# cai4cai/torchsparsegradutils

Hardware: AMD Instinct MI355X
Metric: CSR SpMM+SDDMM achieved HBM GB/s (algorithmic bytes), N=1e6 nnz/row=27 RHS=32, fwd+bwd (higher is better)
Workload: dtype f32

## Files before the change

### include/tsgu_hip.h

```cpp
#ifndef TSGU_HIP_H
#define TSGU_HIP_H

#include <stdint.h>

#ifdef __cplusplus
extern "C" {
#endif

#define TSGU_ABI_VERSION 7

typedef enum {
    TSGU_OK = 0,
    TSGU_ERR_BAD_DTYPE = -1,
    TSGU_ERR_BAD_ARG = -2,
    TSGU_ERR_TOO_LARGE = -3,
    TSGU_ERR_LAUNCH = -4,
    TSGU_ERR_RUNTIME = -5,
    TSGU_ERR_RESERVED_6 = -6,
    TSGU_ERR_TIMEOUT = -7
} tsgu_status;

typedef enum { TSGU_F32 = 0, TSGU_F64 = 1, TSGU_BF16 = 2 } tsgu_vtype;
typedef enum { TSGU_I32 = 0, TSGU_I64 = 1 } tsgu_itype;

int tsgu_abi_version(void);
const char* tsgu_status_string(int status);
int tsgu_device_info(int device, char* name, int cap, int* n_cu, int* wave_size);
int tsgu_device_cu_count(int device, int* n_cu);
int tsgu_device_copy(const void* src, void* dst, int64_t bytes, int device, void* stream);

int tsgu_index_fingerprint(int itype, int64_t n, const void* x, void* out2, int accumulate, int device, void* stream);
int tsgu_index_fingerprint_match(int itype, int64_t n, const void* x, const void* ref, void* copy, void* out3, int accumulate,
                                 int device, void* stream);

int tsgu_csr_spmm(int vtype, int itype,
                  int64_t n_rows, int64_t n_cols, int64_t nnz_per_item,
                  const void* crow, const void* col, const void* val, const void* perm,
                  const void* B, int64_t ldb, int64_t b_col_stride, int64_t b_batch_stride,
                  void* C, int64_t ldc, int64_t c_col_stride, int64_t c_batch_stride,
                  int64_t p, int64_t batch, int64_t max_row_nnz,
                  const void* dot_w, int64_t ldw, void* dot_partial,
                  int device, void* stream);

int64_t tsgu_spmm_num_blocks(int vtype, int64_t n_rows, int64_t nnz_per_item, int64_t p, int64_t max_row_nnz);

int tsgu_csr_geometry(int kernel, int vtype, int64_t n_rows, int64_t nnz_per_item, int64_t p, int64_t max_row_nnz,
                      int wide_ok, int col_strided,
                      int* vec, int* column_lanes, int* entry_lanes, int64_t* column_tiles, int* row_runs, int* stage_entries);

int tsgu_csr_sddmm(int vtype, int itype,
                   int64_t n_rows, int64_t n_cols, int64_t nnz_per_item,
                   const void* crow, const void* col,
                   const void* G, int64_t ldg, int64_t g_batch_stride,
                   const void* B, int64_t ldb, int64_t b_batch_stride,
                   void* out, double alpha, int swap_roles,
                   int64_t p, int64_t batch,
                   int device, void* stream);

int tsgu_coo_sddmm(int vtype, int itype, int64_t nnz,
                   const void* row, const void* col,
                   const void* G, int64_t ldg, const void* B, int64_t ldb,
                   void* out, double alpha, int64_t p,
                   int device, void* stream);

int tsgu_csr_mm_backward(int vtype, int itype, int64_t n_rows, int64_t n_cols, int64_t nnz_per_item,
                         const void* t_ptr, const void* t_idx, const void* t_perm, const void* val,
                         const void* G, int64_t ldg, int64_t g_batch_stride,
                         const void* B, int64_t ldb, int64_t b_batch_stride,
                         void* gradA_vals, void* gradB, int64_t ldgb, int64_t gb_batch_stride,
                         int64_t p, int64_t batch, int device, void* stream);

typedef struct tsgu_rowpack_plan {
    int64_t nblocks;
    int32_t ecap, ucap;
    int32_t nclasses;
    int32_t rows_per_group;
    const void* uptr;
    const void* ucol;
    const void* upos;
    const void* sperm;
    const void* order;
    const void* vpair;
    const void* eptr;
    const void* wcls;
    const void* wbase;
    const void* cne;
    const void* srcstart;
} tsgu_rowpack_plan;

int tsgu_rowpack_geometry(int vtype, int64_t p, int* rows_per_block, int* entry_lanes, int* max_entries, int* max_union,
                          int* lds_budget_bytes);
int tsgu_csr_spmm_rowpack(int vtype, int itype, int64_t n_rows, int64_t n_cols, int64_t nnz, const void* ptr,
                          const tsgu_rowpack_plan* plan, const void* val, const void* B, int64_t ldb, void* C, int64_t ldc,
                          int64_t p, int device, void* stream);
int tsgu_csr_mm_backward_rowpack(int vtype, int itype, int64_t n_rows_t, int64_t n_cols_t, int64_t nnz, const void* t_ptr,
                                 const tsgu_rowpack_plan* plan, const void* val, const void* G, int64_t ldg, const void* B,
                                 int64_t ldb, void* gradA_vals, void* gradB, int64_t ldgb, int64_t p, int device, void* stream);
int tsgu_csr_sddmm_rowpack(int vtype, int itype, int64_t n_rows, int64_t n_cols, int64_t nnz, const void* ptr,
                           const tsgu_rowpack_plan* plan, const void* R, int64_t ldr, const void* Cm, int64_t ldc,
                           void* out_vals, double alpha, int64_t p, int device, void* stream);

typedef struct tsgu_tile_plan {
    int64_t n_rows, n_cols, nnz;
    int64_t n_blocks;
    int32_t rows_per_block, max_union, max_entries, reserved;
    const void* desc;
    const void* ucol;
    const void* lidx;
    const void* rptr;
    const void* cpos;
    const void* cslot;
    const void* ent;
    const void* xrow;
} tsgu_tile_plan;

int tsgu_tile_geometry(int vtype, int64_t p, int* rows_per_block, int* max_union, int* max_entries);
int tsgu_csr_spmm_tile(int vtype, const tsgu_tile_plan* plan, const void* val, const void* B, int64_t ldb, void* C, int64_t ldc,
                       int64_t p, int device, void* stream);
int tsgu_csr_sddmm_tile(int vtype, const tsgu_tile_plan* plan, const void* R, int64_t ldr, const void* Cm, int64_t ldc, void* out_vals,
                        double alpha, int64_t p, int device, void* stream);

typedef struct tsgu_lattice_plan {
    int32_t kind;
    int32_t nb, nx, ny, nz;
    int32_t ry, rz;
    int32_t ncls, recw;
    int32_t nloc;
    int32_t uniform_len;
    int32_t ty, tz;
    int32_t nseg;
    int32_t threads;
    int32_t ring;
    int32_t chunks_per_lane;
    const void* rec;
    const void* lens;
    const void* rcls;
    const void* rstart;
    const void* wlist;
} tsgu_lattice_plan;

int tsgu_lattice_lds_bytes(int mode, int vtype, int64_t p, int ty, int tz, int ry, int rz, int nloc, int recw, int threads, int ring,
                           int chunks_per_lane);
int tsgu_csr_spmm_lattice(int vtype, const tsgu_lattice_plan* plan, int64_t n_rows, int64_t nnz, const void* val,
                          const void* B, int64_t ldb, void* C, int64_t ldc, int64_t p, int device, void* stream);
int tsgu_csr_spmm_lattice_dot(int vtype, const tsgu_lattice_plan* plan, int64_t n_rows, int64_t nnz, const void* val,
                              const void* B, int64_t ldb, void* C, int64_t ldc, int64_t p, void* dot_partial, int64_t dot_rows,
                              const int* skip, const void* dot_w, int device, void* stream);
int tsgu_csr_sddmm_lattice(int vtype, const tsgu_lattice_plan* plan, int64_t n_rows, int64_t nnz, const void* R, int64_t ldr,
                           const void* Cm, int64_t ldc, void* out_vals, double alpha, int64_t p, int device, void* stream);

typedef struct tsgu_march_plan {
    int32_t nb, nx, ny, nz;
    int32_t ry, rz;
    int32_t ntap;
    int32_t tap_dy[9], tap_dz[9];
    int32_t ncls, ident;
    int32_t ty, tz;
    int32_t nseg;
    int32_t threads;
    uint32_t mask;
    int32_t periodic;
    int32_t uniform_len;
    const void* kidx;
    const void* rcls;
    const void* rstart;
} tsgu_march_plan;

int tsgu_march_supported(int mode, int mask, int uniform_len, int threads);
int tsgu_march_lds_bytes(int mode, int vtype, int64_t p, int ty, int tz, int ry, int rz, int ncls, int threads);
int tsgu_csr_spmm_march(int vtype, const tsgu_march_plan* plan, int transposed, int64_t n_rows, int64_t nnz, const void* val,
                        const void* B, int64_t ldb, void* C, int64_t ldc, int64_t p, int device, void* stream);
int tsgu_csr_sddmm_march(int vtype, const tsgu_march_plan* plan, int64_t n_rows, int64_t nnz, const void* R, int64_t ldr,
                         const void* Cm, int64_t ldc, void* out_vals, double alpha, int accumulate, int64_t p, int device,
                         void* stream);

int tsgu_lattice_slots(void);
int tsgu_lattice_rows(int itype, int64_t n_rows, const void* crow, const void* col, int nb, int nx, int ny, int nz, const void* disp, int nd,
                      void* slot, void* thash, void* trep, const void* remap, const void* ctable, const void* lens, void* rcls, void* status,
                      int box_mask, int periodic, int device, void* stream);
int tsgu_lattice_row_codes(int itype, int64_t n_rows, const void* crow, const void* col, int nb, int nx, int ny, int nz, const void* disp,
                           int nd, const void* rows, int nrows, void* out, int device, void* stream);
int tsgu_lattice_block_classes(int64_t n_rows, const void* rcls, int nb, int nx, int ny, int nz, int ty, int tz, int nseg, void* mask,
                               int device, void* stream);

int tsgu_csr_sptrsm(int vtype, int itype,
                    int64_t n, int64_t nnz,
                    const void* ptr, const void* idx, const void* perm, const void* val,
                    int lower, int unit,
                    const void* B, int64_t ldb, int64_t b_col_stride, void* X, int64_t ldx, int64_t p,
                    void* work, int workgroups_per_cu, int device, void* stream);
int64_t tsgu_sptrsm_work_bytes(int64_t n, int64_t p);

typedef struct {
    int32_t kind, nlines, nz, ncls, width, uniform_len, front_lines, reserved;
    const void* tab;
    const void* lens;
    const void* rcls;
    const void* rstart;
} tsgu_trsm_lattice_plan;
int tsgu_csr_sptrsm_lattice(int vtype, const tsgu_trsm_lattice_plan* plan, int64_t nnz, const void* val,
                            int lower, int unit,
                            const void* B, int64_t ldb, int64_t b_col_stride, void* X, int64_t ldx, int64_t p,
                            void* work, int workgroups, int device, void* stream);

int64_t tsgu_cg_fold_rows(void);
int tsgu_cg_alpha(int vtype, const void* pap_partial, int64_t n_partial, void* fold, void* scal, int* flags,
                  double eps, int64_t p, int device, void* stream);
int tsgu_cg_update1(int vtype, int64_t n, int64_t p,
                    void* r, const void* Ap, void* x, const void* pvec,
                    const void* scal, const int* flags, void* rr_partial,
                    int device, void* stream);
int tsgu_cg_update1_alpha(int vtype, int64_t n, int64_t p, void* r, const void* Ap, void* x, const void* pvec, const void* pap_partial,
                          int64_t n_partial, void* scal, const int* flags, double eps, void* rr_partial, int device, void* stream);
int64_t tsgu_cg2_num_blocks(int vtype, int64_t n, int64_t p);
int tsgu_cg2_residual(int vtype, int64_t n, int64_t p, void* r, const void* Ap, const void* pap_partial, int64_t n_partial, void* scal2,
                      const int* flags2, int parity, double eps, void* rr_partial, int device, void* stream);
int tsgu_cg2_direction(int vtype, int64_t n, int64_t p, const void* r, void* pvec, void* x, const void* rr_partial, int64_t n_partial,
                       void* scal2, int* flags2, int parity, double eps, double stop_updating_after, double tolerance,
                       int min_iter_index, void* hist, int n_hist, int device, void* stream);
int64_t tsgu_cg_num_blocks(int vtype, int64_t n, int64_t p);
int tsgu_cg_beta(int vtype, const void* rr_partial, int64_t n_partial, void* scal, int* flags,
                 double eps, double stop_updating_after, double tolerance, int iter_index,
                 int min_iter_index, int64_t p, int device, void* stream);
int tsgu_cg_beta_precond(int vtype, const void* rr_partial, int64_t n_partial, const void* rz_partial, int64_t n_rz, void* scal,
                         int* flags, double eps, double stop_updating_after, double tolerance, int iter_index,
                         int min_iter_index, int64_t p, int device, void* stream);
int tsgu_cg_update2(int vtype, int64_t n, int64_t p, const void* r, void* pvec,
                    const void* scal, const int* flags, int device, void* stream);

int tsgu_bicg_scalar(int vtype, int phase, const void* partial, int64_t n_partial, int64_t set_stride, void* fold,
                     void* scal, int* flags, double abstol, double reltol, int matvec_max, int nmv0, int64_t p,
                     int device, void* stream);
int tsgu_bicg_vector(int vtype, int which, int64_t n, int64_t p, void* a0, void* a1, const void* a2, const void* a3,
                     const void* a4, const void* scal, const int* flags, void* partial, int64_t set_stride,
                     int device, void* stream);
int tsgu_bicg_update_x_precond(int vtype, int64_t n, int64_t p, void* x, void* r, const void* s, const void* t,
                               const void* q, const void* z, const void* scal, const int* flags, void* partial,
                               int device, void* stream);

int tsgu_minres_scalar(int vtype, int phase, const void* partial, int64_t n_partial, int64_t set_stride, void* fold,
                       void* scal, int* flags, double eps, double tol, double shift, int64_t p, int device, void* stream);
int tsgu_minres_vector(int vtype, int which, int64_t n, int64_t p, void* a0, const void* a1, void* a2, const void* a3,
                       void* a4, const void* scal, const int* flags, void* partial, int64_t set_stride, int with_norms,
                       int device, void* stream);
int tsgu_minres_scalar_ms(int vtype, int phase, const void* partial, int64_t n_partial, int64_t set_stride, void* fold,
                          void* scal, int* flags, double eps, double tol, const void* shifts, int n_shift, double value,
                          int64_t p, int device, void* stream);
int tsgu_minres_vector_ms(int vtype, int which, int64_t n, int64_t p, void* a0, const void* a1, void* a2, const void* a3,
                          void* a4, void* qc, const void* scal, const int* flags, void* partial, int64_t set_stride,
                          int with_norms, int n_shift, int64_t shift_stride, double value, int device, void* stream);

int64_t tsgu_coldot_max_blocks(int64_t n, int64_t p);
int tsgu_coldot(int vtype, int64_t n, int64_t p, const void* X, int64_t ldx,
                const void* Y, int64_t ldy, void* partial, void* out,
                int device, void* stream);

int tsgu_segment_logsumexp_workspace(int vtype, int64_t nnz, int64_t* bytes_host);
int tsgu_segment_logsumexp(int vtype, int itype, int64_t n_groups, int64_t nnz, const void* ptr, const void* perm,
                           const void* val, int include_zeros, int64_t axis_len, void* out, int64_t groups_per_item,
                           int64_t item_stride, void* workspace, int64_t workspace_bytes, int device, void* stream);
int tsgu_segment_logsumexp_backward(int vtype, int itype, int64_t nnz, const void* val, const void* ptr, int64_t n_groups,
                                    const void* g_grp, const void* lse_grp, const void* idx, const void* g_idx,
                                    const void* lse_idx, void* grad, int device, void* stream);

int tsgu_segment_mm_tile_rows(void);
int tsgu_segment_mm(int vtype, int itype, int64_t n, int64_t d1, int64_t d2, int64_t n_seg, const void* offsets,
                    const void* tile_ptr, int64_t max_tiles, const void* perm, const void* a, int64_t lda, const void* b,
                    int64_t b_stride0, int64_t b_stride1, int64_t b_stride2, void* out, int64_t ldo, int device, void* stream);
int tsgu_segment_mm_grad_b_workspace(int vtype, int64_t n, int64_t n_seg, int64_t d1, int64_t d2, int64_t* chunk_rows,
                                     int64_t* max_chunks, int64_t* bytes);
int tsgu_segment_mm_grad_b(int vtype, int itype, int64_t n, int64_t d1, int64_t d2, int64_t n_seg, const void* offsets,
                           const void* chunk_ptr, const void* part_ptr, int64_t chunk_rows, int64_t max_chunks, const void* perm,
                           const void* a, int64_t lda, const void* g, int64_t ldg, void* grad_b, void* workspace,
                           int64_t workspace_bytes, int device, void* stream);

int64_t tsgu_mvn_reduce_blocks(int64_t rows_per_item);
int tsgu_csr_diag_positions(int itype, int64_t n_rows, int64_t nnz, const void* crow, const void* col, const void* perm,
                            void* pos, int device, void* stream);
int tsgu_diag_logsum(int vtype, int itype, int64_t n_rows, int64_t rows_per_item, int64_t n_val, const void* pos,
                     const void* val, void* out, void* partial, int64_t partial_elems, int device, void* stream);
int tsgu_diag_logsum_backward(int vtype, int itype, int64_t n_rows, int64_t rows_per_item, int64_t nnz, const void* crow,
                              const void* perm, const void* pos, const void* val, const void* g, void* grad, int fill,
                              int device, void* stream);
int tsgu_quadform(int vtype, int64_t n, int64_t k, const void* Y, int64_t ldy, int64_t y_col_stride, const void* E,
                  int64_t lde, int64_t e_col_stride, const void* w, int w_mode, int64_t rows_per_item, void* out,
                  void* partial, int64_t partial_elems, int device, void* stream);
int tsgu_quadform_backward(int vtype, int64_t n, int64_t k, const void* Y, int64_t ldy, int64_t y_col_stride, const void* E,
                           int64_t lde, int64_t e_col_stride, const void* w, int w_mode, int64_t rows_per_item, const void* g,
                           void* grad_Y, int64_t ldg, int64_t g_col_stride, void* grad_w, int device, void* stream);
int tsgu_csr_row_sumsq(int vtype, int itype, int64_t n_rows, int64_t nnz, int64_t n_w, const void* crow, const void* col,
                       const void* perm, const void* val, const void* w, const void* add, void* out, int device,
                       void* stream);
int tsgu_csr_row_sumsq_backward(int vtype, int itype, int64_t n_rows, int64_t nnz, int64_t n_w, const void* crow,
                                const void* col, const void* perm, const void* val, const void* w, const void* g, void* grad_val,
                                int device, void* stream);

#ifdef __cplusplus
}
#endif
#endif
```

### torchsparsegradutils_amd/_backend.py

```python

from __future__ import annotations

import ctypes
import functools
import os
import sys
import threading
from typing import Optional

import torch

_HERE = os.path.dirname(os.path.abspath(__file__))
LIB_PATH = os.environ.get("TSGU_LIB_PATH") or os.path.join(_HERE, "csrc", "libtsgu_hip.so")

TSGU_F32, TSGU_F64, TSGU_BF16 = 0, 1, 2
TSGU_I32, TSGU_I64 = 0, 1

_VTYPE = {torch.float32: TSGU_F32, torch.float64: TSGU_F64, torch.bfloat16: TSGU_BF16}
_ITYPE = {torch.int32: TSGU_I32, torch.int64: TSGU_I64}

_lib = None
_lib_lock = threading.Lock()

_i64 = ctypes.c_int64
_int = ctypes.c_int
_ptr = ctypes.c_void_p
_dbl = ctypes.c_double

ABI_VERSION = 7

SIGNATURES = {
    "tsgu_abi_version": (_int, []),
    "tsgu_status_string": (ctypes.c_char_p, [_int]),
    "tsgu_device_info": (_int, [_int, ctypes.c_char_p, _int, ctypes.POINTER(_int), ctypes.POINTER(_int)]),
    "tsgu_device_copy": (_int, [_ptr, _ptr, _i64, _int, _ptr]),
    "tsgu_device_cu_count": (_int, [_int, ctypes.POINTER(_int)]),
    "tsgu_index_fingerprint": (_int, [_int, _i64, _ptr, _ptr, _int, _int, _ptr]),
    "tsgu_index_fingerprint_match": (_int, [_int, _i64, _ptr, _ptr, _ptr, _ptr, _int, _int, _ptr]),
    "tsgu_tile_geometry": (_int, [_int, _i64, ctypes.POINTER(_int), ctypes.POINTER(_int), ctypes.POINTER(_int)]),
    "tsgu_csr_spmm_tile": (_int, [_int, _ptr, _ptr, _ptr, _i64, _ptr, _i64, _i64, _int, _ptr]),
    "tsgu_csr_sddmm_tile": (_int, [_int, _ptr, _ptr, _i64, _ptr, _i64, _ptr, _dbl, _i64, _int, _ptr]),
    "tsgu_csr_spmm": (
        _int,
        [_int, _int, _i64, _i64, _i64, _ptr, _ptr, _ptr, _ptr, _ptr, _i64, _i64, _i64, _ptr, _i64, _i64, _i64, _i64, _i64, _i64,
         _ptr, _i64, _ptr, _int, _ptr],
    ),
    "tsgu_spmm_num_blocks": (_i64, [_int, _i64, _i64, _i64, _i64]),
    "tsgu_csr_geometry": (_int, [_int, _int, _i64, _i64, _i64, _i64, _int, _int, ctypes.POINTER(_int), ctypes.POINTER(_int),
                                 ctypes.POINTER(_int), ctypes.POINTER(_i64), ctypes.POINTER(_int), ctypes.POINTER(_int)]),
    "tsgu_csr_sddmm": (
        _int,
        [_int, _int, _i64, _i64, _i64, _ptr, _ptr, _ptr, _i64, _i64, _ptr, _i64, _i64, _ptr, _dbl, _int, _i64, _i64,
         _int, _ptr],
    ),
    "tsgu_coo_sddmm": (_int, [_int, _int, _i64, _ptr, _ptr, _ptr, _i64, _ptr, _i64, _ptr, _dbl, _i64, _int, _ptr]),
    "tsgu_segment_logsumexp_workspace": (_int, [_int, _i64, ctypes.POINTER(_i64)]),
    "tsgu_segment_logsumexp": (
        _int, [_int, _int, _i64, _i64, _ptr, _ptr, _ptr, _int, _i64, _ptr, _i64, _i64, _ptr, _i64, _int, _ptr],
    ),
    "tsgu_segment_logsumexp_backward": (
        _int, [_int, _int, _i64, _ptr, _ptr, _i64, _ptr, _ptr, _ptr, _ptr, _ptr, _ptr, _int, _ptr],
    ),
    "tsgu_segment_mm_tile_rows": (_int, []),
    "tsgu_segment_mm": (
        _int, [_int, _int, _i64, _i64, _i64, _i64, _ptr, _ptr, _i64, _ptr, _ptr, _i64, _ptr, _i64, _i64, _i64, _ptr, _i64, _int, _ptr],
    ),
    "tsgu_segment_mm_grad_b_workspace": (
        _int, [_int, _i64, _i64, _i64, _i64, ctypes.POINTER(_i64), ctypes.POINTER(_i64), ctypes.POINTER(_i64)],
    ),
    "tsgu_segment_mm_grad_b": (
        _int, [_int, _int, _i64, _i64, _i64, _i64, _ptr, _ptr, _ptr, _i64, _i64, _ptr, _ptr, _i64, _ptr, _i64, _ptr, _ptr, _i64,
               _int, _ptr],
    ),
    "tsgu_csr_mm_backward": (
        _int,
        [_int, _int, _i64, _i64, _i64, _ptr, _ptr, _ptr, _ptr, _ptr, _i64, _i64, _ptr, _i64, _i64, _ptr, _ptr, _i64,
         _i64, _i64, _i64, _int, _ptr],
    ),
    "tsgu_minres_scalar": (
        _int,
        [_int, _int, _ptr, _i64, _i64, _ptr, _ptr, _ptr, _dbl, _dbl, _dbl, _i64, _int, _ptr],
    ),
    "tsgu_minres_vector": (
        _int,
        [_int, _int, _i64, _i64, _ptr, _ptr, _ptr, _ptr, _ptr, _ptr, _ptr, _ptr, _i64, _int, _int, _ptr],
    ),
    "tsgu_minres_scalar_ms": (
        _int,
        [_int, _int, _ptr, _i64, _i64, _ptr, _ptr, _ptr, _dbl, _dbl, _ptr, _int, _dbl, _i64, _int, _ptr],
    ),
    "tsgu_minres_vector_ms": (
        _int,
        [_int, _int, _i64, _i64, _ptr, _ptr, _ptr, _ptr, _ptr, _ptr, _ptr, _ptr, _ptr, _i64, _int, _int, _i64, _dbl, _int, _ptr],
    ),
    "tsgu_bicg_update_x_precond": (_int, [_int, _i64, _i64, _ptr, _ptr, _ptr, _ptr, _ptr, _ptr, _ptr, _ptr, _ptr, _int, _ptr]),
    "tsgu_rowpack_geometry": (
        _int,
        [_int, _i64, ctypes.POINTER(_int), ctypes.POINTER(_int), ctypes.POINTER(_int), ctypes.POINTER(_int),
         ctypes.POINTER(_int)],
    ),
    "tsgu_csr_spmm_rowpack": (_int, [_int, _int, _i64, _i64, _i64, _ptr, _ptr, _ptr, _ptr, _i64, _ptr, _i64, _i64, _int, _ptr]),
    "tsgu_csr_mm_backward_rowpack": (
        _int, [_int, _int, _i64, _i64, _i64, _ptr, _ptr, _ptr, _ptr, _i64, _ptr, _i64, _ptr, _ptr, _i64, _i64, _int, _ptr]),
    "tsgu_csr_sddmm_rowpack": (
        _int, [_int, _int, _i64, _i64, _i64, _ptr, _ptr, _ptr, _i64, _ptr, _i64, _ptr, _dbl, _i64, _int, _ptr]),
    "tsgu_lattice_lds_bytes": (_int, [_int, _int, _i64, _int, _int, _int, _int, _int, _int, _int, _int, _int]),
    "tsgu_csr_spmm_lattice": (_int, [_int, _ptr, _i64, _i64, _ptr, _ptr, _i64, _ptr, _i64, _i64, _int, _ptr]),
    "tsgu_csr_spmm_lattice_dot": (_int, [_int, _ptr, _i64, _i64, _ptr, _ptr, _i64, _ptr, _i64, _i64, _ptr, _i64, _ptr, _ptr, _int, _ptr]),
    "tsgu_csr_sddmm_lattice": (_int, [_int, _ptr, _i64, _i64, _ptr, _i64, _ptr, _i64, _ptr, _dbl, _i64, _int, _ptr]),
    "tsgu_march_supported": (_int, [_int, _int, _int, _int]),
    "tsgu_march_lds_bytes": (_int, [_int, _int, _i64, _int, _int, _int, _int, _int, _int]),
    "tsgu_csr_spmm_march": (_int, [_int, _ptr, _int, _i64, _i64, _ptr, _ptr, _i64, _ptr, _i64, _i64, _int, _ptr]),
    "tsgu_csr_sddmm_march": (_int, [_int, _ptr, _i64, _i64, _ptr, _i64, _ptr, _i64, _ptr, _dbl, _int, _i64, _int, _ptr]),
    "tsgu_lattice_slots": (_int, []),
    "tsgu_lattice_rows": (_int, [_int, _i64, _ptr, _ptr, _int, _int, _int, _int, _ptr, _int, _ptr, _ptr, _ptr, _ptr, _ptr, _ptr, _ptr, _ptr,
                                 _int, _int, _int, _ptr]),
    "tsgu_lattice_row_codes": (_int, [_int, _i64, _ptr, _ptr, _int, _int, _int, _int, _ptr, _int, _ptr, _int, _ptr, _int, _ptr]),
    "tsgu_lattice_block_classes": (_int, [_i64, _ptr, _int, _int, _int, _int, _int, _int, _int, _ptr, _int, _ptr]),
    "tsgu_csr_sptrsm": (
        _int,
        [_int, _int, _i64, _i64, _ptr, _ptr, _ptr, _ptr, _int, _int, _ptr, _i64, _i64, _ptr, _i64, _i64, _ptr, _int, _int, _ptr],
    ),
    "tsgu_sptrsm_work_bytes": (_i64, [_i64, _i64]),
    "tsgu_csr_sptrsm_lattice": (_int, [_int, _ptr, _i64, _ptr, _int, _int, _ptr, _i64, _i64, _ptr, _i64, _i64, _ptr, _int, _int, _ptr]),
    "tsgu_cg_fold_rows": (_i64, []),
    "tsgu_cg_alpha": (_int, [_int, _ptr, _i64, _ptr, _ptr, _ptr, _dbl, _i64, _int, _ptr]),
    "tsgu_cg_update1": (_int, [_int, _i64, _i64, _ptr, _ptr, _ptr, _ptr, _ptr, _ptr, _ptr, _int, _ptr]),
    "tsgu_cg_num_blocks": (_i64, [_int, _i64, _i64]),
    "tsgu_cg_beta": (_int, [_int, _ptr, _i64, _ptr, _ptr, _dbl, _dbl, _dbl, _int, _int, _i64, _int, _ptr]),
    "tsgu_cg_beta_precond": (_int, [_int, _ptr, _i64, _ptr, _i64, _ptr, _ptr, _dbl, _dbl, _dbl, _int, _int, _i64, _int, _ptr]),
    "tsgu_cg_update2": (_int, [_int, _i64, _i64, _ptr, _ptr, _ptr, _ptr, _int, _ptr]),
    "tsgu_cg2_num_blocks": (_i64, [_int, _i64, _i64]),
    "tsgu_cg2_residual": (_int, [_int, _i64, _i64, _ptr, _ptr, _ptr, _i64, _ptr, _ptr, _int, _dbl, _ptr, _int, _ptr]),
    "tsgu_cg2_direction": (_int, [_int, _i64, _i64, _ptr, _ptr, _ptr, _ptr, _i64, _ptr, _ptr, _int, _dbl, _dbl, _dbl, _int, _ptr, _int, _int, _ptr]),
    "tsgu_cg_update1_alpha": (_int, [_int, _i64, _i64, _ptr, _ptr, _ptr, _ptr, _ptr, _i64, _ptr, _ptr, _dbl, _ptr, _int, _ptr]),
    "tsgu_bicg_scalar": (_int, [_int, _int, _ptr, _i64, _i64, _ptr, _ptr, _ptr, _dbl, _dbl, _int, _int, _i64, _int, _ptr]),
    "tsgu_bicg_vector": (_int, [_int, _int, _i64, _i64, _ptr, _ptr, _ptr, _ptr, _ptr, _ptr, _ptr, _ptr, _i64, _int, _ptr]),
    "tsgu_coldot_max_blocks": (_i64, [_i64, _i64]),
    "tsgu_coldot": (_int, [_int, _i64, _i64, _ptr, _i64, _ptr, _i64, _ptr, _ptr, _int, _ptr]),
    "tsgu_mvn_reduce_blocks": (_i64, [_i64]),
    "tsgu_csr_diag_positions": (_int, [_int, _i64, _i64, _ptr, _ptr, _ptr, _ptr, _int, _ptr]),
    "tsgu_diag_logsum": (_int, [_int, _int, _i64, _i64, _i64, _ptr, _ptr, _ptr, _ptr, _i64, _int, _ptr]),
    "tsgu_diag_logsum_backward": (_int, [_int, _int, _i64, _i64, _i64, _ptr, _ptr, _ptr, _ptr, _ptr, _ptr, _int, _int, _ptr]),
    "tsgu_quadform": (_int, [_int, _i64, _i64, _ptr, _i64, _i64, _ptr, _i64, _i64, _ptr, _int, _i64, _ptr, _ptr, _i64, _int, _ptr]),
    "tsgu_quadform_backward": (
        _int, [_int, _i64, _i64, _ptr, _i64, _i64, _ptr, _i64, _i64, _ptr, _int, _i64, _ptr, _ptr, _i64, _i64, _ptr, _int, _ptr],
    ),
    "tsgu_csr_row_sumsq": (_int, [_int, _int, _i64, _i64, _i64, _ptr, _ptr, _ptr, _ptr, _ptr, _ptr, _ptr, _int, _ptr]),
    "tsgu_csr_row_sumsq_backward": (_int, [_int, _int, _i64, _i64, _i64, _ptr, _ptr, _ptr, _ptr, _ptr, _ptr, _ptr, _int, _ptr]),
}

SIGNATURES_SOFTMAX = {
    "tsgu_segment_softmax_workspace": (_int, [_int, _i64, ctypes.POINTER(_i64)]),
    "tsgu_segment_softmax": (_int, [_int, _int, _i64, _i64, _ptr, _ptr, _ptr, _int, _ptr, _ptr, _i64, _int, _ptr]),
    "tsgu_segment_softmax_backward": (_int, [_int, _int, _i64, _i64, _ptr, _ptr, _ptr, _ptr, _int, _ptr, _ptr, _i64, _int, _ptr]),
}

SIGNATURES_ATTENTION = {
    "tsgu_csr_attention_supported": (_int, [_int, _int, _int]),
    "tsgu_csr_attention_geometry": (_int, [_int, _int, _int, ctypes.POINTER(_int), ctypes.POINTER(_int), ctypes.POINTER(_int)]),
    "tsgu_csr_attention": (
        _int, [_int, _int, _i64, _i64, _i64, _ptr, _ptr, _ptr, _ptr, _ptr, _i64, _ptr, _i64, _ptr, _i64, _int, _int, _dbl, _ptr, _i64,
               _ptr, _int, _ptr]),
    "tsgu_csr_attention_backward_rows": (
        _int, [_int, _int, _i64, _i64, _i64, _ptr, _ptr, _ptr, _ptr, _ptr, _i64, _ptr, _i64, _ptr, _i64, _ptr, _i64, _ptr, _int, _int,
               _dbl, _ptr, _i64, _ptr, _ptr, _int, _ptr]),
    "tsgu_csr_attention_backward_cols": (
        _int, [_int, _int, _i64, _i64, _i64, _ptr, _ptr, _ptr, _ptr, _ptr, _i64, _ptr, _i64, _ptr, _i64, _ptr, _i64, _ptr, _ptr, _int,
               _int, _dbl, _ptr, _i64, _ptr, _i64, _int, _ptr]),
}

SIGNATURES_MM_REDUCE = {
    "tsgu_csr_spmm_reduce_geometry": (_int, [_int, _i64, ctypes.POINTER(_int), ctypes.POINTER(_int), ctypes.POINTER(_int)]),
    "tsgu_csr_spmm_reduce": (
        _int, [_int, _int, _i64, _i64, _i64, _ptr, _ptr, _ptr, _ptr, _i64, _i64, _int, _ptr, _i64, _ptr, _i64, _int, _ptr]),
    "tsgu_csr_spmm_reduce_backward_values": (
        _int, [_int, _int, _i64, _i64, _i64, _ptr, _ptr, _ptr, _i64, _ptr, _i64, _ptr, _i64, _i64, _ptr, _int, _ptr]),
    "tsgu_csr_spmm_reduce_backward_dense": (
        _int, [_int, _int, _i64, _i64, _i64, _ptr, _ptr, _ptr, _ptr, _ptr, _i64, _ptr, _i64, _i64, _ptr, _i64, _int, _ptr]),
}

SIGNATURES_SPGEMM = {
    "tsgu_spgemm_bins": (_int, [ctypes.POINTER(_int), ctypes.POINTER(_int)]),
    "tsgu_spgemm_row_bound": (_int, [_int, _i64, _i64, _ptr, _ptr, _ptr, _ptr, _int, _ptr]),
    "tsgu_spgemm_symbolic": (
        _int, [_int, _int, _i64, _ptr, _i64, _i64, _i64, _ptr, _ptr, _ptr, _ptr, _ptr, _ptr, _int, _ptr, _ptr, _ptr, _int, _ptr]),
    "tsgu_spgemm_numeric": (
        _int, [_int, _int, _int, _i64, _ptr, _i64, _i64, _i64, _ptr, _ptr, _ptr, _ptr, _ptr, _ptr, _ptr, _ptr, _ptr, _ptr, _int, _ptr]),
    "tsgu_spgemm_grad_a": (
        _int, [_int, _int, _i64, _i64, _i64, _i64, _ptr, _ptr, _ptr, _ptr, _ptr, _ptr, _ptr, _ptr, _ptr, _int, _ptr]),
    "tsgu_spgemm_grad_b": (
        _int, [_int, _int, _i64, _i64, _i64, _i64, _ptr, _ptr, _ptr, _ptr, _ptr, _ptr, _ptr, _ptr, _ptr, _ptr, _int, _ptr]),
}

SIGNATURES_BSR = {
    "tsgu_bsr_mm_geometry": (_int, [_int, _i64, _i64, _i64, ctypes.POINTER(_int), ctypes.POINTER(_int), ctypes.POINTER(_int)]),
    "tsgu_bsr_spmm": (_int, [_int, _int, _i64, _i64, _i64, _i64, _i64, _ptr, _ptr, _ptr, _ptr, _i64, _i64, _ptr, _i64, _int, _ptr]),
    "tsgu_bsr_sddmm": (_int, [_int, _int, _i64, _i64, _i64, _i64, _i64, _ptr, _ptr, _ptr, _i64, _ptr, _i64, _i64, _ptr, _int, _ptr]),
    "tsgu_bsr_spmm_t": (
        _int, [_int, _int, _i64, _i64, _i64, _i64, _i64, _ptr, _ptr, _ptr, _ptr, _ptr, _i64, _i64, _ptr, _i64, _int, _ptr]),
}

SIGNATURES_BSR_ATTENTION = {
    "tsgu_bsr_attention_supported": (_int, [_int, _int, _int, _i64, _i64]),
    "tsgu_bsr_attention_geometry": (_int, [_int, _int, _int, _i64, _i64, ctypes.POINTER(_int), ctypes.POINTER(_int)]),
    "tsgu_bsr_attention": (
        _int, [_int, _int, _i64, _i64, _i64, _i64, _i64, _ptr, _ptr, _ptr, _ptr, _i64, _ptr, _i64, _ptr, _i64, _int, _int, _dbl, _ptr,
               _i64, _ptr, _ptr, _int, _ptr]),
    "tsgu_bsr_attention_backward_rows": (
        _int, [_int, _int, _i64, _i64, _i64, _i64, _i64, _ptr, _ptr, _ptr, _ptr, _i64, _ptr, _i64, _ptr, _i64, _ptr, _i64, _ptr, _i64,
               _ptr, _int, _int, _dbl, _ptr, _i64, _ptr, _ptr, _int, _ptr]),
    "tsgu_bsr_attention_backward_cols": (
        _int, [_int, _int, _i64, _i64, _i64, _i64, _i64, _ptr, _ptr, _ptr, _ptr, _ptr, _i64, _ptr, _i64, _ptr, _i64, _ptr, _i64, _ptr,
               _ptr, _int, _int, _dbl, _ptr, _i64, _ptr, _i64, _int, _ptr]),
}

_FACTOR_ARGS = [_int, _int, _i64, _i64, _ptr, _ptr, _ptr, _ptr, _dbl, _ptr, _ptr, _ptr, _int, _int, _ptr]
SIGNATURES_FACTOR = {
    "tsgu_csr_factor_work_bytes": (_i64, [_i64]),
    "tsgu_csr_factor_geometry": (_int, [_int, ctypes.POINTER(_int), ctypes.POINTER(_int)]),
    "tsgu_csr_ilu0": (_int, list(_FACTOR_ARGS)),
    "tsgu_csr_ic0": (_int, list(_FACTOR_ARGS)),
}

SIGNATURES_FSAI = {
    "tsgu_csr_fsai_geometry": (_int, [_int, ctypes.POINTER(_int), ctypes.POINTER(_int)]),
    "tsgu_csr_fsai": (_int, [_int, _int, _i64, _ptr, _ptr, _ptr, _ptr, _ptr, _i64, _ptr, _ptr, _ptr, _int, _int, _ptr]),
}

ABI = {
    "tsgu_hip.h": SIGNATURES,
    "tsgu_hip_softmax.h": SIGNATURES_SOFTMAX,
    "tsgu_hip_attention.h": SIGNATURES_ATTENTION,
    "tsgu_hip_mm_reduce.h": SIGNATURES_MM_REDUCE,
    "tsgu_hip_spgemm.h": SIGNATURES_SPGEMM,
    "tsgu_hip_bsr.h": SIGNATURES_BSR,
    "tsgu_hip_bsr_attention.h": SIGNATURES_BSR_ATTENTION,
    "tsgu_hip_factor.h": SIGNATURES_FACTOR,
    "tsgu_hip_fsai.h": SIGNATURES_FSAI,
}

SIGNATURES_LOBPCG = {
    "tsgu_tall_geometry": (_int, [_int, _i64, _i64, _i64, ctypes.POINTER(_int), ctypes.POINTER(_int), ctypes.POINTER(_int),
                                  ctypes.POINTER(_i64)]),
    "tsgu_tall_gram": (_int, [_int, _i64, _i64, _i64, _ptr, _i64, _ptr, _i64, _ptr, _i64, _ptr, _i64, _int, _int, _ptr]),
    "tsgu_tall_combine": (_int, [_int, _i64, _int, _ptr, _ptr, _ptr, _int, _ptr, _ptr, _ptr, _ptr, _ptr, _ptr, _int, _int, _ptr]),
    "tsgu_lobpcg_residual": (_int, [_int, _i64, _i64, _ptr, _i64, _ptr, _i64, _ptr, _ptr, _i64, _ptr, _ptr, _i64, _int, _int, _ptr]),
}

STAGED = {"tsgu_hip_lobpcg.h": SIGNATURES_LOBPCG}

SIGNATURES_AMG = {
    "tsgu_amg_geometry": (_int, [ctypes.POINTER(_int), ctypes.POINTER(_int), ctypes.POINTER(_int)]),
    "tsgu_csr_amg_hop": (_int, [_int, _i64, _i64, _ptr, _ptr, _ptr, _ptr, _int, _int, _ptr]),
    "tsgu_amg_mis2_update": (_int, [_int, _i64, _ptr, _ptr, _ptr, _ptr, _int, _ptr]),
    "tsgu_csr_affine_spmm": (_int, [_int, _int, _i64, _i64, _i64, _i64, _ptr, _ptr, _ptr, _ptr, _i64, _ptr, _i64, _ptr, _i64, _ptr, _dbl,
                                    _ptr, _i64, _int, _ptr]),
}

STAGED_AMG = {"tsgu_hip_amg.h": SIGNATURES_AMG}

SIGNATURES_GMRES = {
    "tsgu_gmres_geometry": (_int, [_int, _i64, _i64, ctypes.POINTER(_int), ctypes.POINTER(_int), ctypes.POINTER(_i64),
                                   ctypes.POINTER(_i64)]),
    "tsgu_gmres_project": (_int, [_int, _i64, _i64, _int, _ptr, _ptr, _i64, _ptr, _ptr, _int, _int, _ptr]),
    "tsgu_gmres_subtract": (_int, [_int, _i64, _i64, _int, _ptr, _ptr, _i64, _ptr, _ptr, _ptr, _ptr, _int, _int, _ptr]),
    "tsgu_gmres_scale": (_int, [_int, _i64, _i64, _ptr, _ptr, _ptr, _ptr, _int, _int, _ptr]),
    "tsgu_gmres_scalar": (_int, [_int, _int, _int, _int, _ptr, _i64, _ptr, _ptr, _ptr, _dbl, _dbl, _int, _i64, _int, _ptr]),
    "tsgu_gmres_update": (_int, [_int, _i64, _i64, _int, _ptr, _ptr, _i64, _ptr, _ptr, _int, _ptr]),
}

STAGED_GMRES = {"tsgu_hip_gmres.h": SIGNATURES_GMRES}

SIGNATURES_COLOR = {
    "tsgu_color_geometry": (_int, [ctypes.POINTER(_int)] * 6),
    "tsgu_csr_color_round": (_int, [_int, _i64, _i64, _ptr, _ptr, _i64, _ptr, _ptr, _ptr, _ptr, _ptr, _int, _int, _ptr]),
    "tsgu_csr_color_check": (_int, [_int, _i64, _i64, _ptr, _ptr, _i64, _ptr, _ptr, _ptr, _i64, _ptr, _int, _int, _ptr]),
    "tsgu_csr_color_sweep": (_int, [_int, _int, _int, _i64, _i64, _i64, _i64, _i64, _i64, _ptr, _ptr, _ptr, _ptr, _ptr, _ptr, _ptr, _i64,
                                    _ptr, _ptr, _i64, _ptr, _i64, _ptr, _int, _int, _ptr]),
}

STAGED_COLOR = {"tsgu_hip_color.h": SIGNATURES_COLOR}

SIGNATURES_QUADRATURE = {
    "tsgu_quadrature_geometry": (_int, [ctypes.POINTER(_int), ctypes.POINTER(_i64)]),
    "tsgu_tridiag_quadrature": (_int, [_int, _int, _int, _int, _i64, _ptr, _ptr, _ptr, _ptr, _ptr, _int, _ptr]),
    "tsgu_rademacher_fill": (_int, [_int, _i64, _i64, _i64, _ptr, _int, _ptr]),
}

STAGED_QUADRATURE = {"tsgu_hip_quadrature.h": SIGNATURES_QUADRATURE}

SIGNATURES_CIQ = {
    "tsgu_ciq_geometry": (_int, [_int, _i64, _i64, ctypes.POINTER(_int), ctypes.POINTER(_int), ctypes.POINTER(_i64),
                                 ctypes.POINTER(_i64)]),
    "tsgu_ciq_update": (_int, [_int, _i64, _i64, _int, _ptr, _ptr, _ptr, _ptr, _i64, _ptr, _ptr, _ptr, _ptr, _ptr, _ptr, _int, _ptr]),
    "tsgu_ciq_stop": (_int, [_int, _i64, _int, _ptr, _dbl, _ptr, _ptr, _ptr, _int, _ptr]),
}

STAGED_CIQ = {"tsgu_hip_ciq.h": SIGNATURES_CIQ}

SIGNATURES_EXPM = {
    "tsgu_expm_geometry": (_int, [_int, _i64, _i64, ctypes.POINTER(_int), ctypes.POINTER(_int), ctypes.POINTER(_int),
                                  ctypes.POINTER(_i64), ctypes.POINTER(_i64)]),
    "tsgu_cheb_step": (_int, [_int, _i64, _i64, _ptr, _ptr, _ptr, _dbl, _dbl, _dbl, _ptr, _int, _int, _ptr, _int, _int, _ptr, _int, _ptr]),
    "tsgu_cheb_combine": (_int, [_int, _int, _int, _i64, _i64, _int, _int, _ptr, _ptr, _ptr, _i64, _ptr, _int, _ptr]),
}

STAGED_EXPM = {"tsgu_hip_expm.h": SIGNATURES_EXPM}

SIGNATURES_TOPK = {
    "tsgu_topk_geometry": (_int, [_int, _i64, _int, ctypes.POINTER(_int), ctypes.POINTER(_int), ctypes.POINTER(_int),
                                  ctypes.POINTER(_int), ctypes.POINTER(_int)]),
    "tsgu_topk_mm": (_int, [_int, _ptr, _ptr, _ptr, _i64, _i64, _i64, _int, _dbl, _int, _i64, _ptr, _ptr, _ptr, _int, _i64, _i64, _i64,
                            _i64, _i64, _int, _ptr]),
}

STAGED_TOPK = {"tsgu_hip_topk.h": SIGNATURES_TOPK}


class HipExtensionMissing(RuntimeError):
    pass


def load_library():
    global _lib
    if _lib is not None:
        return _lib
    with _lib_lock:
        if _lib is not None:
            return _lib
        if not os.path.exists(LIB_PATH):
            raise HipExtensionMissing(
                f"{LIB_PATH} not found: build the gfx950 extension first "
                "(python -c 'import __graft_entry__ as g; g.build()' or make -C torchsparsegradutils_amd/csrc). "
                "torchsparsegradutils_amd has no CPU or eager fallback."
            )
        lib = ctypes.CDLL(LIB_PATH, mode=ctypes.RTLD_GLOBAL)
        for table in (*ABI.values(), *STAGED.values(), *STAGED_AMG.values(), *STAGED_GMRES.values(),
                      *STAGED_COLOR.values(), *STAGED_QUADRATURE.values(), *STAGED_CIQ.values(), *STAGED_EXPM.values(),
                      *STAGED_TOPK.values()):
            for name, (res, args) in table.items():
                fn = getattr(lib, name)
                fn.restype = res
                fn.argtypes = args
        if lib.tsgu_abi_version() != ABI_VERSION:
            raise HipExtensionMissing("libtsgu_hip.so ABI version mismatch; rebuild the extension")
        _lib = lib
    return _lib


def check(status: int, what: str) -> None:
    if status != 0:
        msg = load_library().tsgu_status_string(status).decode()
        raise RuntimeError(f"{what} failed: {msg} (tsgu status {status})")


def _query(name: str, *args):
    fn = getattr(load_library(), name)
    outs = [t._type_(0) for t in fn.argtypes[len(args):]]
    check(fn(*args, *map(ctypes.byref, outs)), name)
    return tuple(int(o.value) for o in outs)


def vtype_of(t: torch.Tensor) -> int:
    try:
        return _VTYPE[t.dtype]
    except KeyError:
        raise RuntimeError(f"torchsparsegradutils_amd: unsupported value dtype {t.dtype}") from None


def itype_of(t: torch.Tensor) -> int:
    try:
        return _ITYPE[t.dtype]
    except KeyError:
        raise RuntimeError(f"torchsparsegradutils_amd: unsupported index dtype {t.dtype}") from None


def operand_device(*tensors: torch.Tensor) -> torch.device:
    dev = None
    for t in tensors:
        if t is None:
            continue
        if dev is None:
            dev = t.device
        elif t.device != dev:
            raise RuntimeError(f"all operands must be on the same device, got {dev} and {t.device}")
    return dev


def require_device(*tensors: torch.Tensor) -> torch.device:
    dev = None
    for t in tensors:
        if t is None:
            continue
        if not t.is_cuda:
            raise RuntimeError(
                f"the gfx950 kernels of torchsparsegradutils_amd were handed a tensor on '{t.device}': CPU operands are served by "
                "the torch-op path (_cpu.py) only when ALL operands of a call live on the CPU"
            )
        if dev is None:
            dev = t.device
        elif t.device != dev:
            raise RuntimeError(f"all operands must be on the same device, got {dev} and {t.device}")
    return dev


def _raw_stream(dev: torch.device) -> int:
    return torch._C._cuda_getCurrentRawStream(dev.index)


def launch(name: str, dev: torch.device, *args) -> None:
    fn = getattr(_lib or load_library(), name)
    argv = [a.data_ptr() if isinstance(a, torch.Tensor) else a for a in args]
    if torch.cuda.current_device() == dev.index:
# ... 1601 lines not shown
```

### torchsparsegradutils_amd/_lattice.py

```python

from __future__ import annotations

import ctypes
import os
from typing import Dict, Optional, Tuple

import torch

MAX_CLASSES = 255
MAX_RADIUS = 2
MAX_LEN = 32
PAD_LO = PAD_HI = 0x7FF00
_MODE_SPMM, _MODE_SDDMM, _MODE_SPMMT = 0, 1, 2
PACKED_T = False
_CU_COUNT: Dict[int, int] = {}


def num_cu(device=None) -> int:
    idx = -1
    if device is not None and getattr(device, "type", "cpu") == "cuda":
        idx = device.index if device.index is not None else torch.cuda.current_device()
    if idx not in _CU_COUNT:
        n = 256
        if idx >= 0:
            try:
                from . import _backend

                n = int(_backend.device_cu_count(idx)) or 256
            except Exception:
                n = 256
        _CU_COUNT[idx] = n
    return _CU_COUNT[idx]


class LatticePlan:

    __slots__ = ("kind", "nb", "nx", "ny", "nz", "ry", "rz", "ncls", "recw", "uniform_len", "codes", "ksrc", "lens",
                 "lens_host", "rcls", "rstart", "n_rows", "nnz", "box", "_cfg", "_march", "_trsm")

    def __init__(self):
        self._cfg: Dict[tuple, "LatticeConfig"] = {}
        self.box = None
        self._march = False
        self._trsm = None

    def plan_bytes(self) -> int:
        total = 0
        for t in (self.lens, self.rcls, self.rstart):
            if t is not None:
                total += t.numel() * t.element_size()
        for cfg in self._cfg.values():
            if cfg is not None:
                total += cfg.rec.numel() * cfg.rec.element_size() + cfg.wlist.numel()
        return total


class LatticeConfig:

    __slots__ = ("ty", "tz", "nseg", "threads", "rec", "lds_bytes", "struct", "struct_addr", "wlist", "nloc", "ring", "cpl", "uses", "tuned")


SAMPLE_ROWS = 256


def _clusters_to_dims(pos, n: int) -> Optional[Tuple[int, int]]:
    if not pos:
        return None
    clusters = [[pos[0]]]
    reach = max(pos[0], MAX_RADIUS)
    for o in pos[1:]:
        if o - clusters[-1][-1] <= reach:
            clusters[-1].append(o)
        else:
            reach = clusters[-1][-1] + MAX_RADIUS
            clusters.append([o])
    if clusters[0][0] > MAX_RADIUS:
        clusters.insert(0, [])
    if len(clusters) not in (2, 3) or (clusters[0] and clusters[0][-1] > MAX_RADIUS):
        return None
    lo, hi = clusters[1][0], clusters[1][-1]
    mid = (lo + hi) // 2
    cands = sorted((c for c in range(max(hi - MAX_RADIUS, 2), lo + MAX_RADIUS + 1) if n % c == 0), key=lambda c: abs(c - mid))
    if not cands:
        return None
    nz = cands[0]
    if len(clusters) == 2:
        return nz, nz
    lo, hi = clusters[2][0], clusters[2][-1]
    mid = (lo + hi) // 2
    first = (max(lo - MAX_RADIUS, 2 * nz) + nz - 1) // nz * nz
    cands = sorted((c for c in range(first, hi + MAX_RADIUS + 1, nz) if n % c == 0), key=lambda c: abs(c - mid))
    if not cands:
        return None
    return nz, cands[0]


def _sample_dims(g) -> Optional[Tuple[int, int, int, int]]:
    from collections import Counter

    n = g.n_rows
    m = min(n, SAMPLE_ROWS)
    r0 = max(0, n // 2 - m // 2)

    def sample(first):
        ptr = g.crow[first:first + m + 1].tolist()
        cols = g.col[ptr[0]:ptr[-1]].tolist()
        return ptr, cols

    found = None
    for first in dict.fromkeys((r0, max(0, n // 3 - m // 2), max(0, min(n - m, (2 * n) // 3 + 17 * m)))):
        ptr, cols = sample(first)
        if not cols:
            continue
        cnt = Counter()
        base = ptr[0]
        for i in range(m):
            r = first + i
            cnt.update(abs(c - r) for c in cols[ptr[i] - base:ptr[i + 1] - base])
        found = _clusters_to_dims(sorted(o for o, k in cnt.items() if k * 2 > m and o > 0), n)
        if found is not None and n % found[1] == 0 and n % found[0] == 0:
            break
        found = None
    if found is None:
        return None
    nz, d2 = found
    planes = n // d2
    ptr, cols = sample(0)
    base, mx = ptr[0], 0
    for i in range(m):
        px = i // d2
        for c in cols[ptr[i] - base:ptr[i + 1] - base]:
            mx = max(mx, abs(c // d2 - px))
    nx = planes if mx <= 1 else mx + 1
    if nx < 1 or planes % nx:
        return None
    return planes // nx, nx, d2 // nz, nz


def build_lattice_plan_hip(g, be, forward: Optional[LatticePlan] = None, dims=None) -> Optional[LatticePlan]:
    import numpy as np

    if g.batch is not None or g.perm is not None or g.n_rows != g.n_cols or g.n_rows < 8 or not (1 <= g.nnz < 2**31):
        return None
    n = g.n_rows
    dev = g.crow.device
    kind = 0 if forward is None else 1
    if kind == 1:
        dims = (forward.nb, forward.nx, forward.ny, forward.nz)
        codes = forward.codes
        disp = torch.unique(codes[codes >= 0]).to(torch.uint8).to(dev)
    else:
        disp = None
        if dims is None:
            dims = _sample_dims(g)
        if dims is None:
            return None
    crow, col = g.crow.contiguous(), g.col.contiguous()
    slots = be.load_library().tsgu_lattice_slots()
    NST = 8
    init = np.empty(NST + slots + 2 * slots, dtype=np.int32)
    init[:NST] = 0
    init[NST:NST + slots] = np.iinfo(np.int32).max
    init[NST + slots:].view(np.int64)[:] = np.iinfo(np.int64).min
    work = torch.from_numpy(init).to(dev)
    status, trep, thash = work[:NST], work[NST:NST + slots], work[NST + slots:].view(torch.int64)
    slot = torch.empty(n, dtype=torch.int16, device=dev)
    be.lattice_rows(crow, col, dims, status, slot, thash=thash, trep=trep, disp=disp)
    host = work.cpu().numpy()
    bad, ry, rz, maxlen = (int(v) for v in host[:4])
    if bad or maxlen > MAX_LEN or maxlen < 1:
        return None
    hh = host[NST + slots:].view(np.int64)
    used = np.nonzero(hh != np.iinfo(np.int64).min)[0]
    ncls = used.size
    if ncls > MAX_CLASSES or ncls == 0:
        return None
    order = used[np.argsort(hh[used], kind="stable")]
    remap = np.zeros(slots, dtype=np.uint8)
    remap[order] = np.arange(ncls, dtype=np.uint8)
    rep_host = host[NST:NST + slots][order].astype(np.int64)
    rep = torch.from_numpy(rep_host).to(dev)
    table = torch.empty((ncls, 32), dtype=torch.int32, device=dev)
    be.lattice_row_codes(crow, col, dims, rep, table, disp=disp)
    tab_host = table.cpu()
    lens = torch.from_numpy((tab_host.numpy() >= 0).sum(1).astype(np.uint8)).to(dev)
    rcls = torch.zeros(n + 64, dtype=torch.uint8, device=dev)
    status.zero_()
    box = box_candidate(tab_host.numpy(), rep_host, dims, ry, rz) if kind == 0 else None
    be.lattice_rows(crow, col, dims, status, slot, remap=torch.from_numpy(remap).to(dev), ctable=table, lens=lens, rcls=rcls, disp=disp,
                    box_mask=box[0] if box else 0, periodic=box[1] if box else 0)
    st2 = status.cpu()
    if int(st2[0]) != 0:
        return None
    if box is not None and int(st2[4]) != 0:
        box = None
    tab = tab_host.to(torch.int64)
    cl = (tab >= 0).sum(1)
    if kind == 0:
        uniform = int(cl[0]) if bool((cl == cl[0]).all()) else 0
        if uniform:
            rstart = torch.zeros(4, dtype=torch.int32, device=dev)
        else:
            rstart = (crow if crow.dtype == torch.int32 else crow.to(torch.int32)).clone()
        if dims[2] == 1:
            ry = 0
    else:
        uniform, rstart, ry, rz = forward.uniform_len, forward.rstart, forward.ry, forward.rz
    nb, nx, ny, nz = dims
    recw = (int(cl.max()) + 3) // 4 * 4
    tab = tab[:, :recw].contiguous()
    plan = LatticePlan()
    plan.kind, plan.nb, plan.nx, plan.ny, plan.nz, plan.ry, plan.rz = kind, nb, nx, ny, nz, ry, rz
    plan.ncls, plan.recw, plan.uniform_len = ncls, recw, uniform
    plan.n_rows, plan.nnz = n, g.nnz
    if kind == 1:
        plan.ksrc = torch.where(tab >= 0, tab % 32, tab)
        plan.codes = torch.where(tab >= 0, torch.div(tab, 32, rounding_mode="floor"), tab)
    else:
        plan.codes, plan.ksrc = tab, None
    plan.lens_host = cl
    plan.lens = lens
    plan.rcls = rcls
    plan.rstart = rstart
    plan.box = box
    return plan


def box_candidate(codes, rep_rows, dims, ry: int, rz: int):
    nb, nx, ny, nz = (int(v) for v in dims)
    if min(nx, ny, nz) < 3 or ry > 1 or rz > 1 or len(rep_rows) > MARCH_MAX_CLASSES:
        return None
    mask, periodic = 0, 0
    for row, seq in zip(rep_rows, codes):
        row = int(row)
        z, y, x = row % nz, (row // nz) % ny, (row // (ny * nz)) % nx
        for code in seq:
            code = int(code)
            if code < 0:
                continue
            dz, dy, dx = code % 5 - 2, (code // 5) % 5 - 2, code // 25 - 1
            if abs(dy) > 1 or abs(dz) > 1:
                return None
            mask |= 1 << ((dx + 1) * 9 + (dy + 1) * 3 + dz + 1)
            if not 0 <= x + dx < nx:
                periodic |= 1
            if not 0 <= y + dy < ny:
                periodic |= 2
            if not 0 <= z + dz < nz:
                periodic |= 4
    return (mask, periodic) if mask else None


def workgroup_classes_hip(plan: LatticePlan, ty: int, tz: int, nseg: int, be) -> torch.Tensor:
    import numpy as np

    nb, nx, ny, nz = plan.nb, plan.nx, plan.ny, plan.nz
    nblocks = nb * nseg * -(-ny // ty) * -(-nz // tz)
    dev = plan.rcls.device
    mask = torch.zeros((nblocks, 4), dtype=torch.int64, device=dev)
    be.lattice_block_classes(plan.rcls, plan.n_rows, (nb, nx, ny, nz), ty, tz, nseg, mask)
    bits = np.unpackbits(mask.cpu().numpy().view(np.uint8).reshape(nblocks, 32), axis=1, bitorder="little")
    nloc = int(bits.sum(1).max())
    idx = np.argsort(1 - bits, axis=1, kind="stable")[:, :nloc].astype(np.uint8)
    wl = np.where(np.take_along_axis(bits, idx.astype(np.int64), axis=1) == 1, idx, np.uint8(0xFF))
    return torch.from_numpy(np.ascontiguousarray(wl)).to(dev)


def records(plan: LatticePlan, ty: int, tz: int, row_bytes: int, slot_bytes: int, ring: int = 4, elem_bytes: int = 4) -> torch.Tensor:
    hz = tz + 2 * plan.rz
    hr = (ty + 2 * plan.ry) * hz
    codes = plan.codes
    valid = codes >= 0
    c = torch.where(valid, codes, torch.zeros_like(codes))
    dz = c % 5 - 2
    dy = torch.div(c, 5, rounding_mode="floor") % 5 - 2
    dx = torch.div(c, 25, rounding_mode="floor") - 1
    out = []
    for ph in range(ring):
        slot = (ph + dx) % ring
        lo = slot * (hr * row_bytes) + (dy * hz + dz) * row_bytes
        lo = torch.where(valid, lo, torch.full_like(lo, PAD_LO))
        if plan.kind == 0:
            out.append(lo.to(torch.int32))
        else:
            k = torch.where(valid, plan.ksrc, torch.zeros_like(plan.ksrc))
            if PACKED_T and row_bytes % 128 == 0:
                assert slot_bytes == row_bytes
                out.append(torch.where(valid, lo + k * 4, torch.full_like(lo, PAD_LO)).to(torch.int32))
            else:
                hi = slot * (hr * slot_bytes) + (dy * hz + dz) * slot_bytes + k * elem_bytes
                hi = torch.where(valid, hi, torch.full_like(hi, PAD_HI))
                out.append(torch.stack((lo, hi), -1).to(torch.int32))
    return torch.stack(out, 0).contiguous()


def workgroup_classes(plan: LatticePlan, ty: int, tz: int, nseg: int) -> torch.Tensor:
    nb, nx, ny, nz = plan.nb, plan.nx, plan.ny, plan.nz
    n = plan.n_rows
    dev = plan.rcls.device
    seg_len = -(-nx // nseg)
    tiles_y, tiles_z = -(-ny // ty), -(-nz // tz)
    r = torch.arange(n, device=dev, dtype=torch.int64)
    z = r % nz
    y = torch.div(r, nz, rounding_mode="floor") % ny
    xx = torch.div(r, ny * nz, rounding_mode="floor")
    x = xx % nx
    item = torch.div(xx, nx, rounding_mode="floor")
    blk = ((item * nseg + torch.div(x, seg_len, rounding_mode="floor")) * tiles_y + torch.div(y, ty, rounding_mode="floor")) * tiles_z \
        + torch.div(z, tz, rounding_mode="floor")
    nblocks = nb * nseg * tiles_y * tiles_z
    pairs = torch.unique(blk * 256 + plan.rcls[:n].to(torch.int64))
    pb = torch.div(pairs, 256, rounding_mode="floor")
    counts = torch.bincount(pb, minlength=nblocks)
    nloc = int(counts.max())
    start = torch.zeros(nblocks + 1, dtype=torch.int64, device=dev)
    start[1:] = torch.cumsum(counts, 0)
    within = torch.arange(pairs.numel(), device=dev) - start[pb]
    wl = torch.full((nblocks, nloc), 0xFF, dtype=torch.uint8, device=dev)
    wl[pb, within] = (pairs % 256).to(torch.uint8)
    return wl.contiguous()



_NLOC_GUESS = (8, 27)
_CFG_ENV = os.environ.get("TSGU_LATTICE_CFG", "")


def _candidates(limit: int):
    for ty in (1, 2, 3, 4, 5, 6, 8, 10, 12, 16, 20, 24, 32):
        for tz in (4, 5, 6, 8, 10, 12, 16, 20, 24, 32, 50, 64):
            if ty * tz <= limit:
                yield ty, tz


def choose_config(plan: LatticePlan, mode: int, vtype: int, p: int, elem_bytes: int, lds_bytes_fn) -> Optional[Tuple[int, int, int, int, int]]:
    ranked = rank_configs(plan, mode, vtype, p, elem_bytes, lds_bytes_fn)
    return ranked[0] if ranked else None


def rank_configs(plan: LatticePlan, mode: int, vtype: int, p: int, elem_bytes: int, lds_bytes_fn, keep: int = 6):
    if _CFG_ENV:
        v = [int(t) for t in _CFG_ENV.split(",")]
        return [(v[0], v[1], min(v[2], plan.nx), v[3], (v[4] if len(v) > 4 else 4), (v[5] if len(v) > 5 else 1))]
    cl = p * elem_bytes // 16
    found = {}
    alpha = 0.35 if plan.kind == 0 else 0.8
    for threads in (256, 512, 1024):
        rpp = threads // cl
        for ty, tz in _candidates(rpp):
            if ty > plan.ny or tz > plan.nz or (plan.ny == 1 and ty != 1):
                continue
            if elem_bytes == 8 and tz % 4 and plan.nz >= 8:
                continue
            ring = 4
            lds = lds_bytes_fn(mode, vtype, p, ty, tz, plan.ry, plan.rz, min(plan.ncls, _NLOC_GUESS[plan.kind]), plan.recw, threads, ring)
            if lds <= 0:
                continue
            per_cu = min(160 * 1024 // lds, 2048 // threads)
            if per_cu < 1:
                continue
            nr = ty * tz
            tiles = -(-plan.ny // ty) * -(-plan.nz // tz)
            lane_util = (plan.ny * plan.nz) / (tiles * rpp)
            halo = (ty + 2 * plan.ry) * (tz + 2 * plan.rz) / nr
            slots = num_cu(getattr(getattr(plan, 'rcls', None), 'device', None)) * per_cu
            waves = per_cu * threads // 64
            hide = 1.5 if waves < 16 else (1.0 if per_cu >= 2 else 1.15)
            base = plan.nb * tiles
            for nseg in range(1, min(plan.nx, 64) + 1):
                seg_len = -(-plan.nx // nseg)
                if seg_len * (nseg - 1) >= plan.nx:
                    continue
                nwg = base * nseg
                fill = nwg / (-(-nwg // slots) * slots)
                cost = (1.0 / lane_util) * (1.0 + alpha * (halo - 1.0)) * (1.0 + 2.0 / seg_len) / fill * hide
                key = (ty, tz, threads)
                if key not in found or cost < found[key][0]:
                    found[key] = (cost, (ty, tz, nseg, threads, ring, 1))
    if mode == _MODE_SPMMT and elem_bytes == 2:
        for (ty, tz, threads), (cost, c) in list(found.items()):
            if threads != 256:
                continue
            for more, gain in ((512, 0.92), (1024, 0.85)):
                lds = lds_bytes_fn(mode, vtype, p, ty, tz, plan.ry, plan.rz, min(plan.ncls, _NLOC_GUESS[plan.kind]), plan.recw, more, c[4])
                if lds > 0 and 160 * 1024 // lds < 2:
                    found[(ty, tz, more)] = (cost * gain, (ty, tz, c[2], more, c[4], c[5]))
    return [c for _, c in sorted(found.values())[:keep]]


class _LatticePlanStruct(ctypes.Structure):

    _fields_ = [(k, ctypes.c_int32) for k in ("kind", "nb", "nx", "ny", "nz", "ry", "rz", "ncls", "recw", "nloc", "uniform_len",
                                               "ty", "tz", "nseg", "threads", "ring", "chunks_per_lane")] + [(k, ctypes.c_void_p) for k in ("rec", "lens", "rcls", "rstart", "wlist")]


def build_config(plan: LatticePlan, cand, mode: int, vtype: int, p: int, elem_bytes: int, lds_bytes_fn, be=None) -> Optional[LatticeConfig]:
    ty, tz, nseg, threads, ring, cpl = cand
    wlist = workgroup_classes_hip(plan, ty, tz, nseg, be) if be is not None else workgroup_classes(plan, ty, tz, nseg)
    nloc = wlist.size(1)
    lds = lds_bytes_fn(mode, vtype, p, ty, tz, plan.ry, plan.rz, nloc, plan.recw, threads, ring, cpl)
    if lds <= 0:
        return None
    slot = (plan.recw * (max(4, elem_bytes if elem_bytes == 8 else 4) if mode == _MODE_SDDMM else elem_bytes) + 15) // 16 * 16
    if slot % 64 == 0:
        slot += 16
    if PACKED_T and mode == _MODE_SPMMT and (p * elem_bytes) % 128 == 0:
        slot = p * elem_bytes
    cfg = LatticeConfig()
    cfg.ty, cfg.tz, cfg.nseg, cfg.threads, cfg.lds_bytes = ty, tz, nseg, threads, lds
    cfg.wlist, cfg.nloc, cfg.ring, cfg.cpl = wlist, nloc, ring, cpl
    cfg.uses, cfg.tuned = 0, False
    cfg.rec = records(plan, ty, tz, p * elem_bytes, slot, ring, elem_bytes).to(plan.rcls.device)
    cfg.struct = _LatticePlanStruct(plan.kind, plan.nb, plan.nx, plan.ny, plan.nz, plan.ry, plan.rz, plan.ncls, plan.recw,
                                    nloc, plan.uniform_len, ty, tz, nseg, threads, ring, cpl, cfg.rec.data_ptr(), plan.lens.data_ptr(),
                                    plan.rcls.data_ptr(), plan.rstart.data_ptr(), wlist.data_ptr())
    cfg.struct_addr = ctypes.addressof(cfg.struct)
    return cfg


def config_for(plan: LatticePlan, mode: int, vtype: int, p: int, elem_bytes: int, lds_bytes_fn, be=None) -> Optional[LatticeConfig]:
    key = (mode, vtype, p)
    cfg = plan._cfg.get(key)
    if cfg is None and key not in plan._cfg:
        for cand in rank_configs(plan, mode, vtype, p, elem_bytes, lds_bytes_fn):
            cfg = build_config(plan, cand, mode, vtype, p, elem_bytes, lds_bytes_fn, be)
            if cfg is not None:
                break
        plan._cfg[key] = cfg
    return cfg


TUNE = os.environ.get("TSGU_LATTICE_TUNE", "1") == "1"
TUNE_AFTER_USES = int(os.environ.get("TSGU_LATTICE_TUNE_AFTER", "3"))
TUNE_PER_SIZE = 3
TUNE_MARGIN = 0.93
TUNE_LOG = []


def tune_candidates(plan: LatticePlan, mode: int, vtype: int, p: int, elem_bytes: int, lds_bytes_fn):
    if _CFG_ENV:
        return []
    ranked = rank_configs(plan, mode, vtype, p, elem_bytes, lds_bytes_fn, keep=1 << 30)
    taken, per = [], {}
    for c in ranked:
        if per.get(c[3], 0) < TUNE_PER_SIZE:
            per[c[3]] = per.get(c[3], 0) + 1
            taken.append(c)
    return taken


def tune_config(plan: LatticePlan, mode: int, vtype: int, p: int, elem_bytes: int, lds_bytes_fn, be, time_ms) -> Optional[LatticeConfig]:
    key = (mode, vtype, p)
    cur = plan._cfg.get(key)
    if cur is None:
        return None
    cur.tuned = True
    tried = []
    best, best_ms, cur_ms = cur, None, None
    for cand in tune_candidates(plan, mode, vtype, p, elem_bytes, lds_bytes_fn):
        same = cand == (cur.ty, cur.tz, cur.nseg, cur.threads, cur.ring, cur.cpl)
        cfg = cur if same else build_config(plan, cand, mode, vtype, p, elem_bytes, lds_bytes_fn, be)
        if cfg is None:
            continue
        ms = time_ms(cfg)
        tried.append((cand, ms))
        if same:
            cur_ms = ms
        if best_ms is None or ms < best_ms:
            best, best_ms = cfg, ms
    if cur_ms is not None and best is not cur and best_ms > TUNE_MARGIN * cur_ms:
        best = cur
    best.tuned = True
    best.uses = cur.uses
    plan._cfg[key] = best
    TUNE_LOG.append((plan.kind, mode, vtype, p, tried, (best.ty, best.tz, best.nseg, best.threads, best.ring, best.cpl)))
    return best


ENABLE_MARCH = os.environ.get("TSGU_ENABLE_MARCH", "1") == "1"
ENABLE_MARCH_RAW = os.environ.get("TSGU_MARCH_RAW", "1") != "0"
_MARCH_CFG_ENV = os.environ.get("TSGU_MARCH_CFG", "")
_MARCH_CFG_MODE_ENV = {m: os.environ.get("TSGU_MARCH_CFG_" + n, "") for m, n in ((0, "FWD"), (1, "SDDMM"), (2, "SPMMT"))}
MARCH_TAPS = 9
MARCH_MAX_CLASSES = 64
_MARCH_WAVES_PER_CU = {0: 20, 1: 20, 2: 16}
MARCH_SDDMM_SEGMENT_FACTOR = int(os.environ.get("TSGU_MARCH_SDDMM_SEGMENT_FACTOR", "1"))
_MARCH_THREADS = {0: (256, 512), 1: (256, 512), 2: (512, 256), 3: (256,)}
_MARCH_HALO_COST = {0: 0.1, 1: 0.1, 2: 0.8, 3: 0.8}


class MarchTables:

    __slots__ = ("ident", "taps", "mask", "periodic", "full", "kidx_host", "kidx", "_cfg", "_line_ok")


class MarchConfig:

    __slots__ = ("mode", "ty", "tz", "nseg", "threads", "lds_bytes", "struct", "struct_addr", "ring", "cpl", "nloc", "tables", "col_tile")
    march = True


class _MarchPlanStruct(ctypes.Structure):

    _fields_ = ([(k, ctypes.c_int32) for k in ("nb", "nx", "ny", "nz", "ry", "rz", "ntap")] + [("tap_dy", ctypes.c_int32 * 9), ("tap_dz", ctypes.c_int32 * 9)]
                + [(k, ctypes.c_int32) for k in ("ncls", "ident", "ty", "tz", "nseg", "threads")] + [("mask", ctypes.c_uint32)]
                + [(k, ctypes.c_int32) for k in ("periodic", "uniform_len")] + [(k, ctypes.c_void_p) for k in ("kidx", "rcls", "rstart")])


MARCH_FULL = (1 << 27) - 1


def march_tables(plan: LatticePlan) -> Optional[MarchTables]:
    if plan._march is not False:
        return plan._march
    plan._march = None
    if plan.kind != 0 or plan.box is None or plan.ncls > MARCH_MAX_CLASSES or min(plan.nx, plan.ny, plan.nz) < 3:
        return None
    mask, periodic = plan.box

    def slot_of(code):
        return (code // 25) * 9 + ((code // 5) % 5 - 1) * 3 + code % 5 - 1

    canon = [s for s in range(27) if mask >> s & 1]
    ident = None
    kidx = [[0xFF] * 32 for _ in range(plan.ncls)]
    for c, row in enumerate(plan.codes.tolist()):
        slots = [slot_of(code) for code in row if code >= 0]
        if len(set(slots)) != len(slots) or len(slots) > 27:
            return None
        if slots == canon:
            ident = c
        for k, sl in enumerate(slots):
            kidx[c][sl] = k
        kidx[c][31] = len(slots)
    if ident is None:
        return None
    mt = MarchTables()
    mt.ident, mt.mask, mt.periodic, mt.full = ident, mask, periodic, mask == MARCH_FULL
    mt.taps = [(dy, dz) for dy in (-1, 0, 1) for dz in (-1, 0, 1)]
    mt.kidx_host = torch.tensor(kidx, dtype=torch.uint8)
    mt.kidx = mt.kidx_host.to(plan.rcls.device)
    mt._cfg = {}
    plan._march = mt
    return mt


def march_config_for(plan: LatticePlan, mode: int, vtype: int, p: int, lds_bytes_fn, supported_fn=None) -> Optional[MarchConfig]:
    if not ENABLE_MARCH or vtype != 0 or not (p in (16, 32, 64) or (p > 64 and p % 64 == 0 and p <= 1024)):
        return None
    if p == 16 and mode == 0 and not _MARCH_CFG_ENV:
        return None
    mt = march_tables(plan)
    if mt is None:
        return None
    if mt.full and not plan.uniform_len and 36 * plan.ny * plan.nz >= 1 << 24:
        return None
    key = (mode, p)
    if key in mt._cfg:
        return mt._cfg[key]
    pt = min(p, 64)
    cl = pt // 4
    best = None
    pinned = _MARCH_CFG_MODE_ENV.get(mode) or _MARCH_CFG_ENV
    if pinned:
        v = [int(t) for t in pinned.split(",")]
        cands = [(v[0], v[1], min(v[2], plan.nx), v[3])]
        if supported_fn is not None and not supported_fn(mode, mt.mask, plan.uniform_len, v[3]):
            cands = []
    else:
        cands = []
        for threads in _MARCH_THREADS[mode]:
            if supported_fn is not None and not supported_fn(mode, mt.mask, plan.uniform_len, threads):
                continue
            rpp = threads // cl
            tz = 8
            if rpp // tz >= 1 and rpp // tz <= plan.ny and tz <= plan.nz:
                cands.append((rpp // tz, tz, 0, threads))
    for ty, tz, nseg, threads in cands:
        lds = lds_bytes_fn(mode, vtype, pt, ty, tz, 1, 1, plan.ncls, threads)
        if lds <= 0:
            continue
        per_cu = max(1, min(160 * 1024 // lds, _MARCH_WAVES_PER_CU[mode] * 64 // threads))
        slots = num_cu(getattr(getattr(plan, 'rcls', None), 'device', None)) * per_cu
        tiles = -(-plan.ny // ty) * -(-plan.nz // tz)
        base = plan.nb * tiles
        util = (plan.ny * plan.nz) / (tiles * ty * tz)
        halo = (ty + 2) * (tz + 2) / (ty * tz)
        util /= 1.0 + _MARCH_HALO_COST[mode] * (halo - 1.0)
        choices = [nseg] if nseg else range(1, min(plan.nx, 64) + 1)
        for ns_ in choices:
            seg_len = -(-plan.nx // ns_)
            if seg_len * (ns_ - 1) >= plan.nx:
                continue
            nwg = base * ns_
            cost = -(-nwg // slots) * (seg_len + 5) / util
            if best is None or cost < best[0]:
                best = (cost, ty, tz, ns_, threads, lds)
        if best is not None:
            break
    cfg = None
    if best is not None:
        _, ty, tz, nseg, threads, lds = best
        if mode == 1 and not pinned and MARCH_SDDMM_SEGMENT_FACTOR > 1 and mt.full and plan.uniform_len:
            want = nseg * MARCH_SDDMM_SEGMENT_FACTOR
            if want <= 64 and -(-plan.nx // want) >= 8 and -(-plan.nx // want) * (want - 1) < plan.nx:
                nseg = want
        cfg = MarchConfig()
        cfg.mode, cfg.ty, cfg.tz, cfg.nseg, cfg.threads, cfg.lds_bytes = mode, ty, tz, nseg, threads, lds
        cfg.ring, cfg.cpl, cfg.nloc, cfg.tables, cfg.col_tile = 2, 1, plan.ncls, mt, pt
        dy = (ctypes.c_int32 * 9)(*[t[0] for t in mt.taps])
        dz = (ctypes.c_int32 * 9)(*[t[1] for t in mt.taps])
        periodic = mt.periodic
        if (ENABLE_MARCH_RAW and plan.rcls.is_cuda and mt.full and mt.periodic == 7 and plan.uniform_len == 27
                and (getattr(mt, "_line_ok", None) is not None or not torch.cuda.is_current_stream_capturing()) and linemarch_ok(plan, mt)):
            periodic |= 8
        cfg.struct = _MarchPlanStruct(plan.nb, plan.nx, plan.ny, plan.nz, 1, 1, MARCH_TAPS, dy, dz, plan.ncls, mt.ident,
                                      ty, tz, nseg, threads, mt.mask, periodic, plan.uniform_len, mt.kidx.data_ptr(),
                                      plan.rcls.data_ptr(), plan.rstart.data_ptr())
        cfg.struct_addr = ctypes.addressof(cfg.struct)
    mt._cfg[key] = cfg
    return cfg


ENABLE_LINEMARCH = os.environ.get("TSGU_ENABLE_LINEMARCH", "1") != "0"
LINEMARCH_MODES = tuple(int(t) for t in os.environ.get("TSGU_LINEMARCH_MODES", "0,1,2").split(",") if t)
_LINEMARCH_CFG_ENV = os.environ.get("TSGU_LINEMARCH_CFG", "")
_LINE_RANK = ((2, 0, 1), (0, 1, 2), (1, 2, 0))


def linemarch_ok(plan: LatticePlan, mt: MarchTables) -> bool:
    hit = getattr(mt, "_line_ok", None)
    if hit is not None:
        return hit
    ok = False
    if plan.ncls == 27 and mt.full and mt.periodic == 7 and plan.uniform_len == 27:
        kidx = mt.kidx_host[:, :27].tolist()
        cls_of = {}
        for sx in range(3):
            for sy in range(3):
                for sz in range(3):
                    want = [9 * _LINE_RANK[sx][dx] + 3 * _LINE_RANK[sy][dy] + _LINE_RANK[sz][dz] for dx in range(3) for dy in range(3) for dz in range(3)]
                    if want in kidx:
                        cls_of[(sx, sy, sz)] = kidx.index(want)
        if len(cls_of) == 27 and len(set(cls_of.values())) == 27:
            dev = plan.rcls.device

            def state(n):
                s = torch.ones(n, dtype=torch.long, device=dev)
                s[0], s[n - 1] = 0, 2
                return s

            tab = torch.tensor([[[cls_of[(a, b, c)] for c in range(3)] for b in range(3)] for a in range(3)], dtype=plan.rcls.dtype, device=dev)
            want = tab[state(plan.nx)][:, state(plan.ny)][:, :, state(plan.nz)]
            n_rows = plan.nb * plan.nx * plan.ny * plan.nz
            ok = bool((plan.rcls[:n_rows].view(plan.nb, plan.nx, plan.ny, plan.nz) == want).all().item())
    mt._line_ok = ok
    return ok


def linemarch_config_for(plan: LatticePlan, mode: int, vtype: int, p: int, lds_bytes_fn) -> Optional[MarchConfig]:
    if not ENABLE_LINEMARCH or not ENABLE_MARCH or vtype != 2 or p != 16 or mode not in LINEMARCH_MODES or not plan.rcls.is_cuda:
        return None
    mt = march_tables(plan)
    if mt is None or not mt.full or mt.periodic != 7 or plan.uniform_len != 27 or plan.nz not in (8, 16, 32, 64):
        return None
    key = ("line", mode, p)
    if key in mt._cfg:
        return mt._cfg[key]
    cfg = None
    if torch.cuda.is_current_stream_capturing():
        return None
    if linemarch_ok(plan, mt):
        best = None
        pinned = [int(t) for t in _LINEMARCH_CFG_ENV.split(",")] if _LINEMARCH_CFG_ENV else None
        for threads in (512, 1024, 256):
            if threads % (2 * plan.nz):
                continue
            ty = threads // (2 * plan.nz)
            if pinned:
                if ty != pinned[0]:
                    continue
            if ty > plan.ny or plan.ny % ty:
                continue
            lds = lds_bytes_fn(mode, vtype, p, ty, plan.nz, 1, 1, plan.ncls, threads)
            if lds <= 0:
                continue
            per_cu = max(1, min(160 * 1024 // lds, 2048 // threads))
            slots = num_cu(plan.rcls.device) * per_cu
            base = plan.nb * (plan.ny // ty)
            halo = (ty + 2) / ty
            for ns_ in ([pinned[1]] if pinned else range(1, min(plan.nx, 64) + 1)):
                seg_len = -(-plan.nx // ns_)
                if seg_len * (ns_ - 1) >= plan.nx:
                    continue
                cost = -(-base * ns_ // slots) * (seg_len + 3) * threads * halo
                if best is None or cost < best[0]:
                    best = (cost, ty, ns_, threads, lds)
            if best is not None and not pinned:
                break
        if best is not None:
            _, ty, nseg, threads, lds = best
            cfg = MarchConfig()
            cfg.mode, cfg.ty, cfg.tz, cfg.nseg, cfg.threads, cfg.lds_bytes = mode, ty, plan.nz, nseg, threads, lds
            cfg.ring, cfg.cpl, cfg.nloc, cfg.tables, cfg.col_tile = 2, 1, plan.ncls, mt, p
            dy = (ctypes.c_int32 * 9)(*[t[0] for t in mt.taps])
            dz = (ctypes.c_int32 * 9)(*[t[1] for t in mt.taps])
            cfg.struct = _MarchPlanStruct(plan.nb, plan.nx, plan.ny, plan.nz, 1, 1, MARCH_TAPS, dy, dz, plan.ncls, mt.ident,
                                          ty, plan.nz, nseg, threads, mt.mask, mt.periodic, plan.uniform_len, mt.kidx.data_ptr(),
                                          plan.rcls.data_ptr(), plan.rstart.data_ptr())
            cfg.struct_addr = ctypes.addressof(cfg.struct)
    mt._cfg[key] = cfg
    return cfg


TRSM_USED_LOWER, TRSM_USED_UPPER, TRSM_DIAG, TRSM_INLINE = 1 << 8, 1 << 9, 1 << 10, 1 << 11


class _TrsmLatticePlanStruct(ctypes.Structure):

    _fields_ = [(k, ctypes.c_int32) for k in ("kind", "nlines", "nz", "ncls", "width", "uniform_len", "front_lines", "reserved")] \
        + [(k, ctypes.c_void_p) for k in ("tab", "lens", "rcls", "rstart")]


class TrsmTables:

    __slots__ = ("lower", "tab_host", "tab", "front_lines", "struct", "struct_addr")


def _class_extents(plan: LatticePlan):
    n, nx, ny, nz = plan.n_rows, plan.nx, plan.ny, plan.nz
    dev = plan.rcls.device
    r = torch.arange(n, device=dev, dtype=torch.int64)
    coords = torch.stack((torch.div(r, ny * nz, rounding_mode="floor") % nx, torch.div(r, nz, rounding_mode="floor") % ny, r % nz))
    idx = plan.rcls[:n].to(torch.int64).unsqueeze(0).expand(3, n)
    lo = torch.full((3, plan.ncls), 1 << 30, dtype=torch.int64, device=dev).scatter_reduce_(1, idx, coords, "amin")
    hi = torch.full((3, plan.ncls), -1, dtype=torch.int64, device=dev).scatter_reduce_(1, idx, coords, "amax")
    both = torch.stack((lo, hi)).cpu().tolist()
    return both[0], both[1]


def _front_lines(nb: int, nx: int, ny: int, nz: int, sx: int, sy: int) -> int:
    import numpy as np

    start = np.sort((sx * np.arange(nx)[:, None] + sy * np.arange(ny)[None, :]).ravel())
    return int(nb * (np.arange(1, start.size + 1) - np.searchsorted(start, start - nz, side="right")).max())


def trsm_tables(plan: Optional[LatticePlan], lower: bool) -> Optional[TrsmTables]:
    if plan is None:
        return None
    if plan._trsm is None:
        plan._trsm = _trsm_tables_both(plan)
    return plan._trsm[bool(lower)]


def _trsm_tables_both(plan: LatticePlan):
    import numpy as np

    none = {True: None, False: None}
    nb, nx, ny, nz = plan.nb, plan.nx, plan.ny, plan.nz
    if plan.ncls < 1 or plan.ncls > MAX_CLASSES or plan.recw > MAX_LEN or plan.n_rows != nb * nx * ny * nz or plan.n_rows >= 2**31:
        return none
    if plan.kind == 1 and plan.ksrc is None:
        return none
    fixed = (plan.ncls * plan.recw * 8 + plan.ncls * 4 + 15) // 16 * 16
    if fixed + 4 * (plan.recw * 8 + 64 * 8 + 16) > 64 * 1024:
        return none
    lo, hi = _class_extents(plan)
    dims = (nx, ny, nz)
    codes = plan.codes.tolist()
    ksrc = plan.ksrc.tolist() if plan.kind == 1 else None
    W = plan.recw
    tab = np.zeros((plan.ncls, W, 2), dtype=np.int32)
    ok = {True: True, False: True}
    skew = {True: [None, None], False: [None, None]}
    for c in range(plan.ncls):
        if lo[0][c] > hi[0][c]:
            continue
        recs = []
        for k, code in enumerate(codes[c]):
            if code < 0:
                continue
            d = (code // 25 - 1, (code // 5) % 5 - 2, code % 5 - 2)
            eff, wraps = [], False
            for a in range(3):
                da, na = d[a], dims[a]
                if da == 0 or (lo[a][c] + da >= 0 and hi[a][c] + da < na):
                    eff.append(da)
                elif da < 0 and hi[a][c] + da < 0:
                    eff.append(da + na)
                    wraps = True
                elif da > 0 and lo[a][c] + da >= na:
                    eff.append(da - na)
                    wraps = True
                else:
                    return none
            off = (eff[0] * ny + eff[1]) * nz + eff[2]
            if off == 0:
                flags = TRSM_DIAG
            else:
                low = off < 0
                flags = TRSM_USED_LOWER if low else TRSM_USED_UPPER
                if wraps:
                    ok[low] = False
                elif eff[0] == 0 and eff[1] == 0:
                    flags |= TRSM_INLINE
                else:
                    sgn = -1 if low else 1
                    sk = skew[low]
                    if eff[0] == 0:
                        sk[0] = max(sk[0] if sk[0] is not None else -9, sgn * -eff[2])
                    else:
                        cand = (sgn * -eff[1], sgn * -eff[2])
                        sk[1] = cand if sk[1] is None else (max(sk[1][0], cand[0]), max(sk[1][1], cand[1]))
            pos = ksrc[c][k] if plan.kind == 1 else k
            if not 0 <= pos < 32:
                return none
            recs.append((off, pos | flags))
        if plan.kind == 1:
            recs.sort(key=lambda t: t[0])
            if any(a[0] == b[0] for a, b in zip(recs, recs[1:])):
                return none
        if len(recs) != int(plan.lens_host[c]) or len(recs) > W:
            return none
        for k, (off, info) in enumerate(recs):
            tab[c, k, 0], tab[c, k, 1] = off, info
    out = {}
    dev = plan.rcls.device
    tab_dev = None
    for low in (True, False):
        if not ok[low]:
            out[low] = None
            continue
        sy = 0 if skew[low][0] is None else max(skew[low][0] + 1, 0)
        sx = 0 if skew[low][1] is None else max(skew[low][1][1] + 1 + sy * max(skew[low][1][0], 0), 1)
        if tab_dev is None:
            tab_dev = torch.from_numpy(tab).to(dev)
        t = TrsmTables()
        t.lower, t.tab_host, t.tab = low, tab, tab_dev
        t.front_lines = _front_lines(nb, nx, ny, nz, sx, sy)
        t.struct = _TrsmLatticePlanStruct(plan.kind, nb * nx * ny, nz, plan.ncls, W, plan.uniform_len, t.front_lines, 0, tab_dev.data_ptr(),
                                          plan.lens.data_ptr(), plan.rcls.data_ptr(), plan.rstart.data_ptr())
        t.struct_addr = ctypes.addressof(t.struct)
        out[low] = t
    return out
```

### torchsparsegradutils_amd/csrc/march.hip

```cpp
#include "linemarch_impl.h"
#include "march_sets.h"

using namespace tsgu;

namespace tsgu {
int linemarch_fill(LineParams& P, const tsgu_march_plan* pl, int mode, int64_t p, int64_t n_rows, int64_t nnz);
int linemarch_run(int mode, const LineParams& P, int threads, hipStream_t stream);
}

namespace {

int march_lanes(int vtype, int64_t p) {
    if (vtype != TSGU_F32 || p <= 0 || (p * 4) % 16) return 0;
    const int64_t cl = p * 4 / 16;
    return (cl == 4 || cl == 8 || cl == 16) ? (int)cl : 0;
}

int fill(MarchParams& P, const tsgu_march_plan* pl, int mode, int vtype, int64_t p, int64_t n_rows, int64_t nnz, int& cl) {
    if (!pl || n_rows < 0 || nnz < 0) return TSGU_ERR_BAD_ARG;
    cl = march_lanes(vtype, p);
    if (cl == 0) return TSGU_ERR_BAD_DTYPE;
    if (pl->ntap != 9 || pl->ry != 1 || pl->rz != 1) return TSGU_ERR_BAD_ARG;
    if (pl->nb <= 0 || pl->nx < 3 || pl->ny < 3 || pl->nz < 3 || pl->nseg <= 0 || pl->nseg > pl->nx) return TSGU_ERR_BAD_ARG;
    if (!lattice_has_rows(*pl, n_rows)) return TSGU_ERR_BAD_ARG;
    if (pl->mask == 0 || pl->mask >= (1u << 27) || pl->uniform_len < 0 || pl->uniform_len > 27) return TSGU_ERR_BAD_ARG;
    if (pl->uniform_len > 0 ? (int64_t)pl->uniform_len * n_rows != nnz : (pl->rstart == nullptr && pl->mask != kBoxAll)) return TSGU_ERR_BAD_ARG;
    if (pl->mask == kBoxAll && pl->uniform_len == 0) {
        auto line = [](int n, int per) -> int64_t { return per ? 3 * (int64_t)n : 3 * (int64_t)n - 2; };
        if (pl->nb * line(pl->nx, pl->periodic & 1) * line(pl->ny, pl->periodic & 2) * line(pl->nz, pl->periodic & 4) != nnz) return TSGU_ERR_BAD_ARG;
        if (36 * (int64_t)pl->ny * pl->nz >= (1 << 24)) return TSGU_ERR_TOO_LARGE;
    }
    if (pl->threads != 256 && pl->threads != 512) return TSGU_ERR_BAD_ARG;
    if (!pl->kidx || !pl->rcls || pl->ncls <= 0 || pl->ncls > kMarchMaxCls || pl->ident < 0 || pl->ident >= pl->ncls) return TSGU_ERR_BAD_ARG;
    if (nnz > 0x7fffffffLL || n_rows > 0x7fffffffLL || nnz * 4 + 16 > 0xffffffffLL) return TSGU_ERR_TOO_LARGE;
    P.nb = pl->nb, P.nx = pl->nx, P.ny = pl->ny, P.nz = pl->nz;
    P.ty = pl->ty, P.tz = pl->tz, P.ry = pl->ry, P.rz = pl->rz;
    P.tiles_y = (pl->ny + pl->ty - 1) / pl->ty;
    P.tiles_z = (pl->nz + pl->tz - 1) / pl->tz;
    if (!split_x(P, *pl)) return TSGU_ERR_BAD_ARG;
    P.ncls = pl->ncls, P.ident = pl->ident;
    P.mask = pl->mask;
    P.per_x = pl->periodic & 1, P.per_y = pl->periodic >> 1 & 1, P.per_z = pl->periodic >> 2 & 1;
    P.uniform = pl->uniform_len;
    P.raw = (pl->periodic & 8) != 0 && (pl->periodic & 7) == 7 && pl->mask == kBoxAll && pl->uniform_len == 27;
    P.rstart = static_cast<const int*>(pl->rstart);
    const int hz = pl->tz + 2 * pl->rz;
    for (int i = 0; i < 9; ++i) {
        if (pl->tap_dy[i] < -1 || pl->tap_dy[i] > 1 || pl->tap_dz[i] < -1 || pl->tap_dz[i] > 1) return TSGU_ERR_BAD_ARG;
        if (pl->tap_dy[i] != -pl->tap_dy[8 - i] || pl->tap_dz[i] != -pl->tap_dz[8 - i]) return TSGU_ERR_BAD_ARG;
        P.tap_row[i] = pl->tap_dy[i] * hz + pl->tap_dz[i];
    }
    P.kidx = static_cast<const unsigned char*>(pl->kidx);
    P.rcls = static_cast<const unsigned char*>(pl->rcls);
    P.nnz = nnz;
    const int rc = march_layout(P, mode, cl, pl->threads, pl->ntap);
    if (rc < 0) return rc;
    return set_workgroups(P, (int64_t)P.nb * P.nseg * P.tiles_y * P.tiles_z);
}

template <int MODE>
int dispatch(int cl, int threads, const MarchParams& P, void* stream) {
    hipStream_t s = static_cast<hipStream_t>(stream);
    const bool uni = P.uniform > 0;
    if (!march_supported(MODE, P.mask, uni, threads)) return TSGU_ERR_BAD_ARG;
    if (P.mask == kBoxAll) return march_run_box(MODE, cl, threads, uni, P, s);
    const int rc = (P.mask & ~kMarchLowerIncl) == 0 ? march_run_lower(cl, P, s) : march_run_upper(cl, P, s);
    return rc == kMarchNotMine ? TSGU_ERR_BAD_ARG : rc;
}

}

extern "C" {

int tsgu_march_supported(int mode, int mask, int uniform_len, int threads) {
    if (mode < 0 || mode > kLatSpmmT || mask <= 0 || mask > (int)kBoxAll) return 0;
    return march_supported(mode, (uint32_t)mask, uniform_len > 0, threads) ? 1 : 0;
}

int tsgu_march_lds_bytes(int mode, int vtype, int64_t p, int ty, int tz, int ry, int rz, int ncls, int threads) {
    if (vtype == TSGU_BF16) {
        if (mode < 0 || mode > kLatSpmmT || p != 16 || ry != 1 || rz != 1) return TSGU_ERR_BAD_DTYPE;
        LineParams L{};
        L.nz = tz, L.ty = ty, L.ny = ty;
        return linemarch_layout(L, threads, mode);
    }
    const int cl = march_lanes(vtype, p);
    if (cl == 0 || mode < 0 || mode > kLatSpmmT) return TSGU_ERR_BAD_DTYPE;
    if (threads != 256 && threads != 512) return TSGU_ERR_BAD_ARG;
    MarchParams P{};
    P.ty = ty, P.tz = tz, P.ry = ry, P.rz = rz, P.ncls = ncls;
    return march_layout(P, mode, cl, threads, 9);
}

int tsgu_csr_spmm_march(int vtype, const tsgu_march_plan* plan, int transposed, int64_t n_rows, int64_t nnz, const void* val,
                        const void* B, int64_t ldb, void* C, int64_t ldc, int64_t p, int device, void* stream) {
    if (vtype == TSGU_BF16) {
        LineParams L{};
        const int lds = linemarch_fill(L, plan, transposed ? kLatSpmmT : kLatSpmm, p, n_rows, nnz);
        if (lds < 0) return lds;
        if (n_rows == 0) return TSGU_OK;
        if (!val || !aligned16(val) || !lanes_ok({{B, ldb}, {C, ldc}}, p, 8)) return TSGU_ERR_BAD_ARG;
        if (!planes_fit({{B, ldb}}, (int64_t)plan->ny * plan->nz * 2)) return TSGU_ERR_TOO_LARGE;
        if (const int rc = set_device(device)) return rc;
        L.val = val, L.S = B, L.lds_ = ldb, L.out = C, L.ldo = ldc;
        return linemarch_run(transposed ? kLatSpmmT : kLatSpmm, L, plan->threads, static_cast<hipStream_t>(stream));
    }
    MarchParams P{};
    int cl = 0;
    const int mode = transposed ? kLatSpmmT : kLatSpmm;
    if (const int rc = fill(P, plan, mode, vtype, p, n_rows, nnz, cl)) return rc;
    if (n_rows == 0) return TSGU_OK;
    if (!val || !lanes_ok({{B, ldb}, {C, ldc}}, p, 4)) return TSGU_ERR_BAD_ARG;
    if (const int rc = set_device(device)) return rc;
    if (!planes_fit({{B, ldb}, {C, ldc}}, (int64_t)plan->ny * plan->nz * 4)) return TSGU_ERR_TOO_LARGE;
    P.val = val;
    P.S = B;
    P.lds_ = ldb;
    P.out = C;
    P.ldo = ldc;
    return transposed ? dispatch<kLatSpmmT>(cl, plan->threads, P, stream) : dispatch<kLatSpmm>(cl, plan->threads, P, stream);
}

int tsgu_csr_sddmm_march(int vtype, const tsgu_march_plan* plan, int64_t n_rows, int64_t nnz, const void* R, int64_t ldr, const void* Cm,
                         int64_t ldc, void* out_vals, double alpha, int accumulate, int64_t p, int device, void* stream) {
    if (vtype == TSGU_BF16) {
        if (accumulate) return TSGU_ERR_BAD_ARG;
        LineParams L{};
        const int lds = linemarch_fill(L, plan, kLatSddmm, p, n_rows, nnz);
        if (lds < 0) return lds;
        if (n_rows == 0) return TSGU_OK;
        if (!out_vals || !aligned16(out_vals) || !lanes_ok({{R, ldr}, {Cm, ldc}}, p, 8)) return TSGU_ERR_BAD_ARG;
        if (!planes_fit({{R, ldr}, {Cm, ldc}}, (int64_t)plan->ny * plan->nz * 2)) return TSGU_ERR_TOO_LARGE;
        if (const int rc = set_device(device)) return rc;
        L.Own = R, L.ldown = ldr, L.S = Cm, L.lds_ = ldc, L.gvals = out_vals, L.alpha = (float)alpha;
        return linemarch_run(kLatSddmm, L, plan->threads, static_cast<hipStream_t>(stream));
    }
    MarchParams P{};
    int cl = 0;
    if (const int rc = fill(P, plan, kLatSddmm, vtype, p, n_rows, nnz, cl)) return rc;
    if (n_rows == 0) return TSGU_OK;
    if (!out_vals || !lanes_ok({{R, ldr}, {Cm, ldc}}, p, 4)) return TSGU_ERR_BAD_ARG;
    if (const int rc = set_device(device)) return rc;
    if (!planes_fit({{R, ldr}, {Cm, ldc}}, (int64_t)plan->ny * plan->nz * 4)) return TSGU_ERR_TOO_LARGE;
    P.Own = R;
    P.ldown = ldr;
    P.S = Cm;
    P.lds_ = ldc;
    P.gvals = out_vals;
    P.alpha = (float)alpha;
    P.accumulate = accumulate != 0;
    return dispatch<kLatSddmm>(cl, plan->threads, P, stream);
}

}
```

### torchsparsegradutils_amd/csrc/march_box.hip

```cpp
#include "march_sets.h"

namespace tsgu {
int march_run_box(int mode, int cl, int threads, bool uni, const MarchParams& P, hipStream_t s) {
    return march_both_sizes<kBoxAll>(mode, cl, threads, uni, P, s);
}
}
```

### torchsparsegradutils_amd/csrc/march_impl.h

```cpp
#pragma once

#include <type_traits>

#include "lattice_impl.h"

namespace tsgu {

constexpr int kMarchMaxCls = 64;
constexpr int kMarchND = 3;

struct MarchParams {
    int nb, nx, ny, nz;
    int ty, tz, ry, rz;
    int tiles_y, tiles_z;
    int nseg, seg_len;
    int ncls, ident;
    int tap_row[9];
    unsigned mask;
    int per_x, per_y, per_z;
    int uniform;
    const int* rstart;
    int accumulate;
    int raw;
    const unsigned char* kidx;
    const unsigned char* rcls;
    const void* val;
    int64_t nnz;
    const void* S;
    int64_t lds_;
    const void* Own;
    int64_t ldown;
    void* out;
    int64_t ldo;
    void* gvals;
    float alpha;
    int64_t nblocks;
    int o_vals, o_stage, o_tab, o_rows, lds_bytes;
};

template <bool NT_POLICY>
__device__ __forceinline__ void lat_dma4(const void* sbase64, uint32_t voff, unsigned lds_wave_base) {
    unsigned keep;
    if constexpr (NT_POLICY)
        asm volatile("s_mov_b32 %0, m0\n\ts_mov_b32 m0, %3\n\ts_nop 0\n\tglobal_load_lds_dword %1, %2 nt\n\ts_mov_b32 m0, %0"
                     : "=&s"(keep) : "v"(voff), "s"(sbase64), "s"(lds_wave_base) : "memory");
    else
        asm volatile("s_mov_b32 %0, m0\n\ts_mov_b32 m0, %3\n\ts_nop 0\n\tglobal_load_lds_dword %1, %2\n\ts_mov_b32 m0, %0"
                     : "=&s"(keep) : "v"(voff), "s"(sbase64), "s"(lds_wave_base) : "memory");
}

template <int I, int N, typename F>
__device__ __forceinline__ void lat_static_for(F&& f) {
    if constexpr (I < N) {
        f(std::integral_constant<int, I>{});
        lat_static_for<I + 1, N>(f);
    }
}

template <int CTRL>
__device__ __forceinline__ float lat_pair_sum(bool odd, float a0, float a1) {
    const float u = odd ? a1 : a0, w = odd ? a0 : a1;
    return u + dpp_move<CTRL>(w);
}
template <int N>
__device__ __forceinline__ float group_sum_t8(float d0, float d1, float d2, float d3, float d4, float d5, float d6, float d7, int c) {
    static_assert(N >= 1 && N <= 8, "one value per lane of the group");
    const bool b0 = (c & 1) != 0, b1 = (c & 2) != 0, b2 = (c & 4) != 0;
    const float t0 = N > 1 ? lat_pair_sum<0xB1>(b0, d0, d1) : d0 + dpp_move<0xB1>(d0);
    const float t1 = N > 3 ? lat_pair_sum<0xB1>(b0, d2, d3) : (N > 2 ? d2 + dpp_move<0xB1>(d2) : 0.f);
    const float t2 = N > 5 ? lat_pair_sum<0xB1>(b0, d4, d5) : (N > 4 ? d4 + dpp_move<0xB1>(d4) : 0.f);
    const float t3 = N > 7 ? lat_pair_sum<0xB1>(b0, d6, d7) : (N > 6 ? d6 + dpp_move<0xB1>(d6) : 0.f);
    const float r0 = N > 2 ? lat_pair_sum<0x4E>(b1, t0, t1) : t0 + dpp_move<0x4E>(t0);
    const float r1 = N > 6 ? lat_pair_sum<0x4E>(b1, t2, t3) : (N > 4 ? t2 + dpp_move<0x4E>(t2) : 0.f);
    const float lo = r0 + dpp_move<0x104>(r0);
    if constexpr (N <= 4) return lo;
    const float hi = r1 + dpp_move<0x114>(r1);
    return b2 ? hi : lo;
}

constexpr uint32_t kBoxAll = (1u << 27) - 1u;

enum MarchRows { kRowsPointer = 0, kRowsUniform = 1, kRowsBox = 2, kRowsRaw = 3 };

template <typename V, int CL, int MODE, int NT, int NTAP, uint32_t MASK, int ROWS>
__global__ __launch_bounds__(NT, 4) void march_kernel(const MarchParams P) {
    constexpr bool PTR = ROWS == kRowsPointer, RAWR = ROWS == kRowsRaw, UNIF = ROWS == kRowsUniform || RAWR, BOXA = ROWS == kRowsBox;
    static_assert(!RAWR || (MASK == kBoxAll && MODE != kLatSddmm), "raw value rows: SpMM / SpMMT of the whole box");
    static_assert(!BOXA || MASK == kBoxAll, "row starts by box arithmetic: the whole box only");
    constexpr bool FULL = MASK == kBoxAll;
    static_assert(MASK != 0 && MASK <= kBoxAll, "a displacement set of the 3 x 3 x 3 box");
    static_assert(sizeof(V) == 4, "fp32 values and operands");
    constexpr int RB = CL * 16;
    constexpr int NG = NT / CL;
    constexpr int RPW = kWave / CL;
    constexpr int NS = 3 * NTAP;
    constexpr int SLOTS = (NS + 3) / 4 * 4;
    constexpr int VP = SLOTS * 4;
    constexpr int VL = SLOTS / 4;
    constexpr int NGI = (RPW * SLOTS + kWave - 1) / kWave;
    constexpr int NPASS = MODE == kLatSpmmT ? 2 : 1;
    constexpr int RJ = (NS + CL - 1) / CL;
    constexpr int NF = (RPW * VL + kWave - 1) / kWave;
    static_assert(NT % kWave == 0 && kWave % CL == 0 && VP % 64 != 0 && NS < 31, "geometry");

    extern __shared__ uint4 lat_smem[];
    char* const sm = reinterpret_cast<char*>(lat_smem);
    const unsigned sbase = lat_lds_addr(lat_smem);

    const int tid = threadIdx.x;
    const int lane = tid % kWave;
    const int wave = __builtin_amdgcn_readfirstlane(tid / kWave);
    const int c = tid % CL;
    const int g = tid / CL;

    const int HZ = P.tz + 2 * P.rz, HY = P.ty + 2 * P.ry, HR = HY * HZ, NR = P.ty * P.tz;
    const int PB = HR * RB;
    const int plane_rows = P.ny * P.nz;
    auto wrap = [](int v, int m) { return v >= m ? v - m : v; };
    auto has = [](int bit) -> bool { return ((MASK >> bit) & 1u) != 0; };
    constexpr uint32_t mask = MASK;

    const int64_t vblock = xcd_chunked_block(blockIdx.x, P.nblocks);
    int64_t vb = vblock;
    const int tzi = (int)(vb % P.tiles_z);
    vb /= P.tiles_z;
    const int tyi = (int)(vb % P.tiles_y);
    vb /= P.tiles_y;
    const int seg = (int)(vb % P.nseg);
    const int item = (int)(vb / P.nseg);
    const int xs = seg * P.seg_len;
    const int L = P.seg_len < P.nx - xs ? P.seg_len : P.nx - xs;
    const int y0 = tyi * P.ty, z0 = tzi * P.tz;
    const int item_row0 = item * P.nx * plane_rows;
    auto row_of_x = [&](int x) -> int { return item_row0 + x * plane_rows; };
    auto x_ok = [&](int s) -> bool { return P.per_x || (unsigned)(xs - 1 + s) < (unsigned)P.nx; };
    auto halo_row = [&](int hy, int hz) -> int {
        const int yy = y0 - P.ry + hy, zz = z0 - P.rz + hz;
        const bool in = (P.per_y || (unsigned)yy < (unsigned)P.ny) && (P.per_z || (unsigned)zz < (unsigned)P.nz);
        return in ? lat_mod(yy, P.ny) * P.nz + lat_mod(zz, P.nz) : -1;
    };

    auto cnt1 = [](int t, int n, int per) -> int { return per ? 3 : 3 - (t == 0) - (t == n - 1); };
    auto pre1 = [](int t, int per) -> int { return per ? 3 * t : 3 * t - (t > 0); };
    const int boxLz = pre1(P.nz, P.per_z) - (P.per_z ? 0 : 1), boxLy = pre1(P.ny, P.per_y) - (P.per_y ? 0 : 1);
    const int boxLyz = boxLy * boxLz, boxLtot = (pre1(P.nx, P.per_x) - (P.per_x ? 0 : 1)) * boxLyz;
    auto row_const = [&](int r) -> int {
        if constexpr (BOXA) {
            const int y = r / P.nz, z = r - y * P.nz;
            return boxLz * pre1(y, P.per_y) + cnt1(y, P.ny, P.per_y) * pre1(z, P.per_z);
        } else {
            return r;
        }
    };
    auto plane_cx = [&](int x) -> int {
        if constexpr (BOXA) return cnt1(x, P.nx, P.per_x);
        else return FULL ? NS : P.uniform;
    };
    auto plane_base = [&](int x) -> int {
        if constexpr (BOXA) return item * boxLtot + boxLyz * pre1(x, P.per_x);
        else return row_of_x(x) * (FULL ? NS : P.uniform);
    };

    const int staged_rows = MODE == kLatSpmmT ? HR : NR;
    {
        const int* src = reinterpret_cast<const int*>(P.kidx);
        int* dst = reinterpret_cast<int*>(sm + P.o_tab);
        for (int i = tid; i < P.ncls * 8; i += NT) dst[i] = src[i];
        int* rows = reinterpret_cast<int*>(sm + P.o_rows);
        for (int r = tid; r < staged_rows; r += NT) {
            int v;
            if constexpr (MODE == kLatSpmmT) {
                const int hy = r / HZ, hz = r - hy * HZ;
                v = halo_row(hy, hz);
            } else {
                const int ly = r / P.tz, lz = r - ly * P.tz;
                v = (y0 + ly < P.ny && z0 + lz < P.nz) ? (y0 + ly) * P.nz + z0 + lz : -1;
            }
            rows[r] = v;
        }
    }
    __syncthreads();
    const unsigned char* const kidx_s = reinterpret_cast<const unsigned char*>(sm + P.o_tab);
    const int* const rows_s = reinterpret_cast<const int*>(sm + P.o_rows);
    constexpr bool rawv = RAWR;
    auto xrank = [&](int x, int d) -> int { return x == 0 ? (d < 0 ? 2 : d) : (x == P.nx - 1 ? (d > 0 ? 0 : d + 2) : d + 1); };

    const uint32_t ldsb = (uint32_t)P.lds_ * 4u;
    uint32_t roff[kMarchND];
    const int ring_pieces = HR * CL;
#pragma unroll
    for (int d = 0; d < kMarchND; ++d) {
        const int e = d * NT + tid;
        const int hr = e / CL;
        const int hy = hr / HZ, hz = hr - hy * HZ;
        const int hrow_in_plane = e < ring_pieces ? halo_row(hy, hz) : -1;
        roff[d] = hrow_in_plane >= 0 ? (uint32_t)hrow_in_plane * ldsb + (uint32_t)c * 16u : kLatNone;
    }
    if (!(P.per_y && P.per_z)) {
#pragma unroll
        for (int d = 0; d < kMarchND; ++d) {
            const int e = d * NT + tid;
            if (e < ring_pieces && roff[d] == kLatNone) {
                lat_smem[e] = make_uint4(0, 0, 0, 0);
                lat_smem[HR * CL + e] = make_uint4(0, 0, 0, 0);
            }
        }
        if constexpr (MODE == kLatSpmmT) {
            for (int e = tid; e < HR * VL; e += NT) {
                if (rows_s[e / VL] < 0) {
                    *reinterpret_cast<uint4*>(sm + P.o_vals + e * 16) = make_uint4(0, 0, 0, 0);
                    *reinterpret_cast<uint4*>(sm + P.o_vals + HR * VP + e * 16) = make_uint4(0, 0, 0, 0);
                }
            }
        }
        if constexpr (MODE == kLatSpmm) {
            for (int e = tid; e < NR * SLOTS; e += NT) {
                const int r = e / SLOTS, slot = e - r * SLOTS;
                const int ry_ = r / P.tz, rz_ = r - ry_ * P.tz;
                const int yy = y0 + ry_ + (slot / 3) % 3 - 1, zz = z0 + rz_ + slot % 3 - 1;
                const bool beyond = (!P.per_y && (unsigned)yy >= (unsigned)P.ny) || (!P.per_z && (unsigned)zz >= (unsigned)P.nz);
                if (slot < NS && beyond) {
#pragma unroll
                    for (int vbi = 0; vbi < 4; ++vbi) *reinterpret_cast<float*>(sm + P.o_vals + vbi * NR * VP + e * 4) = 0.f;
                }
            }
        }
    }
    const int ly = g / P.tz, lz = g - ly * P.tz;
    const bool ok = g < NR && y0 + ly < P.ny && z0 + lz < P.nz;
    const int crow = ok ? (y0 + ly) * P.nz + z0 + lz : -1;
    const int hrow = (ly + P.ry) * HZ + lz + P.rz;
    const uint32_t coo = (uint32_t)(ok ? crow : 0) * ((uint32_t)P.ldo * 4u) + (uint32_t)c * 16u;
    const uint32_t cown = (uint32_t)(ok ? crow : 0) * ((uint32_t)P.ldown * 4u) + (uint32_t)c * 16u;
    const int cen = hrow * RB + c * 16;

    int srow[NPASS];
    uint32_t foff[NPASS][NF];
    if constexpr (MODE != kLatSddmm) {
#pragma unroll
        for (int q = 0; q < NPASS; ++q) {
            const int r = q * NG + g;
            srow[q] = r < staged_rows ? rows_s[r] : -1;
#pragma unroll
            for (int f = 0; f < NF; ++f) {
                const int piece = f * kWave + lane;
                const int fr = q * NG + wave * RPW + piece / VL;
                const int frow = (piece < RPW * VL && fr < staged_rows) ? rows_s[fr] : -1;
                if constexpr (BOXA) foff[q][f] = frow >= 0 ? (uint32_t)row_const(frow) * 4u : kLatNone;
                else foff[q][f] = frow >= 0 ? (uint32_t)frow * (uint32_t)(NS * 4) + (uint32_t)(piece % VL) * 16u : kLatNone;
            }
        }
    }

    uint32_t fpo[NF];
#pragma unroll
    for (int f = 0; f < NF; ++f) fpo[f] = (uint32_t)((f * kWave + lane) % VL) * 16u;
    int gconst[BOXA ? NPASS : 1][BOXA ? NGI : 1];
    if constexpr (BOXA && MODE != kLatSddmm) {
#pragma unroll
        for (int q = 0; q < NPASS; ++q) {
#pragma unroll
            for (int n = 0; n < NGI; ++n) {
                const int rw = (n * kWave + lane) / SLOTS;
                const int fr = q * NG + wave * RPW + rw;
                const int rr = (rw < RPW && fr < staged_rows) ? rows_s[fr] : -1;
                gconst[q][n] = row_const(rr > 0 ? rr : 0);
            }
        }
    }

    int mid_plain = 0;
    int gk[PTR ? 1 : NPASS][PTR ? 1 : NGI];
    if constexpr (MODE != kLatSddmm && !PTR && !RAWR) {
        const int prow_mid = row_of_x(1);
#pragma unroll
        for (int q = 0; q < NPASS; ++q) {
            const int first = q * NG + wave * RPW;
            const int cm = srow[q] >= 0 ? (int)P.rcls[prow_mid + srow[q]] : P.ident;
            if (FULL && __builtin_amdgcn_ballot_w64(srow[q] >= 0 && cm != P.ident) == 0) mid_plain |= 1 << q;
            const bool allid = !FULL && __builtin_amdgcn_ballot_w64(srow[q] >= 0 && cm != P.ident) == 0;
#pragma unroll
            for (int n = 0; n < NGI; ++n) {
                const int e = n * kWave + lane;
                const int rw = e / SLOTS, slot = e - rw * SLOTS;
                const int rc = __builtin_amdgcn_ds_bpermute((rw < RPW ? rw * CL : 0) * 4, cm);
                const int rr = (rw < RPW && first + rw < staged_rows) ? rows_s[first + rw] : -1;
                const int k = allid ? __builtin_popcount(mask & ((1u << (slot & 31)) - 1u)) : (int)kidx_s[rc * 32 + (slot & 31)];
                const bool want = first < staged_rows && rr >= 0 && slot < NS && has(slot) && k != 0xFF;
                gk[q][n] = !want ? -1 : (UNIF ? (FULL ? NS : P.uniform) * rr + k : k);
            }
        }
    }

    const char* const Sb = static_cast<const char*>(P.S);
    const char* const valb = static_cast<const char*>(P.val);
    const uint32_t val_bytes = (uint32_t)(P.nnz * 4);

    auto dma_ring = [&](int prow, int slot) {
        const char* const pbase = Sb + (int64_t)prow * ldsb;
        const unsigned base = sbase + (unsigned)(slot * PB) + (unsigned)(wave * kWave * 16);
#pragma unroll
        for (int d = 0; d < kMarchND; ++d) {
            if (d * NT < ring_pieces) {
                if (roff[d] != kLatNone) lat_dma16<false>(pbase, roff[d], base + (unsigned)(d * NT * 16));
            }
        }
    };
    auto stage_vals = [&](int pbase, int pcx, bool mid, int xv, unsigned region, const int (&cls)[NPASS], const int (&stt)[NPASS]) {
        if constexpr (MODE != kLatSddmm) {
#pragma unroll
            for (int q = 0; q < NPASS; ++q) {
                const int first = q * NG + wave * RPW;
                if (first < staged_rows) {
                    const unsigned wbase = sbase + region + (unsigned)(first * VP);
                    const bool plain = FULL && (rawv ? (MODE == kLatSpmmT || mid)
                                                     : (!PTR && mid ? (mid_plain >> q & 1) != 0
                                                                    : __builtin_amdgcn_ballot_w64(srow[q] >= 0 && cls[q] != P.ident) == 0));
                    if (plain) {
#pragma unroll
                        for (int f = 0; f < NF; ++f) {
                            uint32_t fo = foff[q][f];
                            if constexpr (UNIF) {
                                if (fo != kLatNone) fo += (uint32_t)pbase * 4u;
                            } else if constexpr (BOXA) {
                                if (fo != kLatNone) fo = __umul24((uint32_t)pcx, fo) + ((uint32_t)pbase * 4u + fpo[f]);
                            } else {
                                const int piece = f * kWave + lane;
                                const int rw = piece / VL;
                                const int rs = __builtin_amdgcn_ds_bpermute((rw < RPW ? rw * CL : 0) * 4, stt[q]);
                                if (fo != kLatNone) fo = (uint32_t)rs * 4u + (uint32_t)(piece % VL) * 16u;
                            }
                            if (fo != kLatNone) {
                                if (__builtin_expect(fo + 16u <= val_bytes, 1)) {
                                    lat_dma16<MODE == kLatSpmm>(valb, fo, wbase + (unsigned)(f * kWave * 16));
                                } else {
                                    float* dst = reinterpret_cast<float*>(sm + region + first * VP + (f * kWave + lane) * 16);
#pragma nounroll
                                    for (int e = 0; e < 4; ++e)
                                        dst[e] = fo + (e + 1) * 4 <= val_bytes ? *reinterpret_cast<const float*>(valb + fo + e * 4) : 0.f;
                                }
                            }
                        }
                    } else if (!PTR && !rawv && mid) {
#pragma unroll
                        for (int n = 0; n < NGI; ++n) {
                            const int gkn = gk[PTR ? 0 : q][PTR ? 0 : n];
                            uint32_t src;
                            if constexpr (BOXA) src = (uint32_t)(pbase + gkn) * 4u + __umul24((uint32_t)pcx, (uint32_t)gconst[q][n]) * 4u;
                            else src = (uint32_t)(pbase + gkn) * 4u;
                            if (gkn >= 0) lat_dma4<MODE == kLatSpmm>(valb, src, wbase + (unsigned)(n * kWave * 4));
                        }
                    } else {
                        const bool allid = !FULL && __builtin_amdgcn_ballot_w64(srow[q] >= 0 && cls[q] != P.ident) == 0;
#pragma unroll
                        for (int n = 0; n < NGI; ++n) {
                            const int e = n * kWave + lane;
                            const int rw = e / SLOTS, slot = e - rw * SLOTS;
                            const int src_lane = (rw < RPW ? rw * CL : 0) * 4;
                            const int rc = __builtin_amdgcn_ds_bpermute(src_lane, cls[q]);
                            const int rr = (rw < RPW && first + rw < staged_rows) ? rows_s[first + rw] : -1;
                            int rs;
                            if constexpr (PTR) rs = __builtin_amdgcn_ds_bpermute(src_lane, stt[q]);
                            else if constexpr (BOXA) rs = pbase + (int)__umul24((uint32_t)pcx, (uint32_t)gconst[q][n]);
                            else rs = pbase + pcx * (rr > 0 ? rr : 0);
                            int k = allid ? __builtin_popcount(mask & ((1u << (slot & 31)) - 1u)) : (int)kidx_s[rc * 32 + (slot & 31)];
                            if (rawv) k = NTAP * xrank(xv, slot / NTAP - 1) + slot % NTAP;
                            if (rr >= 0 && slot < NS && has(slot) && (UNIF || k != 0xFF))
                                lat_dma4<MODE == kLatSpmm>(valb, (uint32_t)rs * 4u + (uint32_t)k * 4u, wbase + (unsigned)(n * kWave * 4));
                        }
                    }
                }
            }
        }
    };
    auto load_cls = [&](int prow, int (&cls)[NPASS], int (&stt)[NPASS]) {
        if constexpr (MODE != kLatSddmm) {
            const unsigned char* const cbase = P.rcls + prow;
#pragma unroll
            for (int q = 0; q < NPASS; ++q) {
                cls[q] = P.ident;
                if constexpr (PTR) stt[q] = 0;
                if (srow[q] >= 0) {
                    cls[q] = cbase[(uint32_t)srow[q]];
                    if constexpr (PTR) stt[q] = P.rstart[prow + srow[q]];
                }
            }
        }
    };
    auto pin_cls = [&](int (&cls)[NPASS], int (&stt)[NPASS]) {
#pragma unroll
        for (int q = 0; q < NPASS; ++q) {
            lat_pin(cls[q]);
            if constexpr (PTR) lat_pin(stt[q]);
        }
    };

    int tapb[NTAP];
#pragma unroll
    for (int i = 0; i < NTAP; ++i) tapb[i] = P.tap_row[i] * RB;
    int tapl[NTAP], tvq[NTAP];
#pragma unroll
    for (int i = 0; i < NTAP; ++i) tapl[i] = tapb[i], tvq[i] = 4 * (NTAP - 1 - i);
    if constexpr (RAWR) {
        {
            const int prow_mid = row_of_x(1);
            if constexpr (MODE == kLatSpmm) {
                const int cm = crow >= 0 ? (int)P.rcls[prow_mid + crow] : P.ident;
#pragma unroll
                for (int i = 0; i < NTAP; ++i) {
                    const int q = (int)kidx_s[cm * 32 + NTAP + i] - NTAP;
#pragma unroll
                    for (int t = 0; t < NTAP; ++t) tapl[t] = q == t ? tapb[i] : tapl[t];
                }
            } else {
#pragma unroll
                for (int i = 0; i < NTAP; ++i) {
                    const int sr = crow >= 0 ? rows_s[hrow + P.tap_row[i]] : -1;
                    const int cs = sr >= 0 ? (int)P.rcls[prow_mid + sr] : P.ident;
                    tvq[i] = 4 * ((int)kidx_s[cs * 32 + NTAP + (NTAP - 1 - i)] - NTAP);
                }
            }
        }
    }
    int tapx[8];
    if constexpr (MODE == kLatSddmm && MASK == kBoxAll && CL == 8 && NTAP == 9) {
#pragma unroll
        for (int i = 0; i < 8; ++i) {
            tapx[i] = tapb[0];
#pragma unroll
            for (int t = 1; t < 8; ++t) tapx[i] = (i ^ c) == t ? tapb[t] : tapx[i];
        }
    }

    auto as4 = [](const uint4& raw, float (&f)[4]) {
        f[0] = __uint_as_float(raw.x), f[1] = __uint_as_float(raw.y), f[2] = __uint_as_float(raw.z), f[3] = __uint_as_float(raw.w);
    };

    int x_ring = lat_mod(xs - 1, P.nx);

    if constexpr (MODE == kLatSpmm || MODE == kLatSpmmT) {
        constexpr int VB = MODE == kLatSpmm ? 4 : 2;
        const int vbuf = (MODE == kLatSpmm ? NR : HR) * VP;
        int x_val = MODE == kLatSpmm ? xs : x_ring;
        int vbase = PTR ? 0 : plane_base(x_val), vcx = PTR ? 0 : plane_cx(x_val);
        auto is_mid = [&](int x) -> bool { return !PTR && x >= 1 && x <= P.nx - 2; };
        auto next_val_plane = [&]() {
            if constexpr (BOXA) vbase += boxLyz * vcx;
            else if constexpr (UNIF) vbase += plane_rows * (FULL ? NS : P.uniform);
            x_val = wrap(x_val + 1, P.nx);
            if constexpr (!PTR) {
                if (x_val == 0) vbase = plane_base(0);
                if constexpr (BOXA) vcx = cnt1(x_val, P.nx, P.per_x);
            }
        };
        int cls[NPASS], cld[NPASS], stt[NPASS], std_[NPASS];
        const int first_val = MODE == kLatSpmm ? 1 : 0;
        const int last_val = MODE == kLatSpmm ? L : L + 1;
#pragma unroll
        for (int q = 0; q < NPASS; ++q) cls[q] = cld[q] = P.ident, stt[q] = std_[q] = 0;
        if (x_ok(first_val) && !is_mid(x_val)) {
            load_cls(row_of_x(x_val), cls, stt);
            pin_cls(cls, stt);
        }
        if (x_ok(0)) dma_ring(row_of_x(x_ring), 0);
        if (x_ok(first_val)) stage_vals(vbase, vcx, is_mid(x_val), x_val, (unsigned)(P.o_vals + (MODE == kLatSpmm ? 1 : 0) * vbuf), cls, stt);
        x_ring = wrap(x_ring + 1, P.nx);
        next_val_plane();
        const int first_next = first_val + 1;
        if (first_next <= last_val && x_ok(first_next) && !is_mid(x_val)) load_cls(row_of_x(x_val), cld, std_);
        lat_step_sync();

        float accP[4], accC[4], accN[4], done[4];
#pragma unroll
        for (int v = 0; v < 4; ++v) accP[v] = accC[v] = accN[v] = done[v] = 0.f;
        int x_out = xs;
        const uint32_t ldob = (uint32_t)P.ldo * 4u;
        auto flush = [&]() {
            if (crow >= 0) {
                char* const obase = static_cast<char*>(P.out) + (int64_t)row_of_x(x_out) * ldob;
                typedef float f4v __attribute__((ext_vector_type(4)));
                const f4v o = {done[0], done[1], done[2], done[3]};
                __builtin_nontemporal_store(o, reinterpret_cast<f4v*>(obase + coo));
            }
            x_out = wrap(x_out + 1, P.nx);
        };
        for (int s = 0; s <= L + 1; ++s) {
            pin_cls(cld, std_);
#pragma unroll
            for (int q = 0; q < NPASS; ++q) cls[q] = cld[q], stt[q] = std_[q];
            if (s >= 3) flush();
            if (s + 1 <= L + 1 && x_ok(s + 1)) dma_ring(row_of_x(x_ring), (s + 1) & 1);
            const int vnext = MODE == kLatSpmm ? s + 2 : s + 1;
            if (vnext <= last_val && x_ok(vnext)) stage_vals(vbase, vcx, is_mid(x_val), x_val, (unsigned)(P.o_vals + (vnext & (VB - 1)) * vbuf), cls, stt);
            x_ring = wrap(x_ring + 1, P.nx);
            next_val_plane();
            if (vnext + 1 <= last_val && x_ok(vnext + 1) && !is_mid(x_val)) load_cls(row_of_x(x_val), cld, std_);
#pragma unroll
            for (int v = 0; v < 4; ++v) accN[v] = 0.f;
            if (crow >= 0 && x_ok(s)) {
                const char* const bb = sm + (s & 1) * PB + cen;
                if constexpr (MODE == kLatSpmm) {
                    const char* const vrow = sm + P.o_vals + g * VP;
                    const char* const vp[3] = {vrow + ((s + 1) & 3) * vbuf, vrow + (s & 3) * vbuf, vrow + ((s - 1) & 3) * vbuf};
                    constexpr int kF0 = 0, kF1 = NTAP / 4, kF2 = 2 * NTAP / 4;
                    constexpr int kN0 = (NTAP - 1) / 4 - kF0 + 1, kN1 = (2 * NTAP - 1) / 4 - kF1 + 1, kN2 = (3 * NTAP - 1) / 4 - kF2 + 1;
                    constexpr int kNA = kN0 > kN1 ? (kN0 > kN2 ? kN0 : kN2) : (kN1 > kN2 ? kN1 : kN2);
                    float a[3][kNA * 4];
                    constexpr int first[3] = {kF0, kF1, kF2}, count[3] = {kN0, kN1, kN2};
#pragma unroll
                    for (int p = 0; p < 3; ++p) {
#pragma unroll
                        for (int m = 0; m < count[p]; ++m) {
                            const uint4 w = *reinterpret_cast<const uint4*>(vp[p] + (first[p] + m) * 16);
                            a[p][4 * m] = __uint_as_float(w.x), a[p][4 * m + 1] = __uint_as_float(w.y);
                            a[p][4 * m + 2] = __uint_as_float(w.z), a[p][4 * m + 3] = __uint_as_float(w.w);
                        }
                    }
                    if constexpr (FULL) {
                        uint4 b[NTAP];
                        constexpr int kAhead = 3;
#pragma unroll
                        for (int i = 0; i < kAhead && i < NTAP; ++i) b[i] = *reinterpret_cast<const uint4*>(bb + tapl[i]);
#pragma unroll
                        for (int i = 0; i < NTAP; ++i) {
                            if (i + kAhead < NTAP) b[i + kAhead] = *reinterpret_cast<const uint4*>(bb + tapl[i + kAhead]);
                            asm volatile("" ::: "memory");
                            float f[4];
                            as4(b[i], f);
                            const float a0 = a[0][i - 4 * first[0]], a1 = a[1][NTAP + i - 4 * first[1]], a2 = a[2][2 * NTAP + i - 4 * first[2]];
#pragma unroll
                            for (int v = 0; v < 4; ++v) {
                                accN[v] = fmaf(a0, f[v], accN[v]);
                                accC[v] = fmaf(a1, f[v], accC[v]);
                                accP[v] = fmaf(a2, f[v], accP[v]);
                            }
                        }
                    } else {
                        uint4 b[NTAP];
#pragma unroll
                        for (int i = 0; i < NTAP; ++i) {
                            b[i] = make_uint4(0, 0, 0, 0);
                            if (has(i) || has(NTAP + i) || has(2 * NTAP + i)) {
                                b[i] = *reinterpret_cast<const uint4*>(bb + tapb[i]);
                            }
                        }
#pragma unroll
                        for (int i = 0; i < NTAP; ++i) {
                            float f[4];
                            as4(b[i], f);
                            const float a0 = a[0][i - 4 * first[0]], a1 = a[1][NTAP + i - 4 * first[1]], a2 = a[2][2 * NTAP + i - 4 * first[2]];
                            if (has(i)) {
#pragma unroll
                                for (int v = 0; v < 4; ++v) accN[v] = fmaf(a0, f[v], accN[v]);
                            }
                            if (has(NTAP + i)) {
#pragma unroll
                                for (int v = 0; v < 4; ++v) accC[v] = fmaf(a1, f[v], accC[v]);
                            }
                            if (has(2 * NTAP + i)) {
#pragma unroll
                                for (int v = 0; v < 4; ++v) accP[v] = fmaf(a2, f[v], accP[v]);
                            }
                        }
                    }
                } else {
                    const char* const vb0 = sm + P.o_vals + (s & 1) * vbuf + hrow * VP;
                    int tapv[NTAP], tvl[NTAP];
#pragma unroll
                    for (int i = 0; i < NTAP; ++i) tapv[i] = P.tap_row[i] * VP, tvl[i] = tapv[i] + tvq[i];
                    if constexpr (FULL) {
                        auto taps = [&](auto rot, int oN, int oC, int oP) {
                            constexpr bool ROT = decltype(rot)::value;
                            uint4 b[NTAP];
                            float a[NTAP][3];
                            constexpr int kAhead = 2;
                            auto fetch = [&](int i) {
                                b[i] = *reinterpret_cast<const uint4*>(bb + tapb[i]);
                                const char* const vr = vb0 + tvl[i];
                                if constexpr (ROT) {
                                    a[i][0] = *reinterpret_cast<const float*>(vr + oN), a[i][1] = *reinterpret_cast<const float*>(vr + oC);
                                    a[i][2] = *reinterpret_cast<const float*>(vr + oP);
                                } else {
#pragma unroll
                                    for (int p = 0; p < 3; ++p) a[i][p] = *reinterpret_cast<const float*>(vr + (2 - p) * (NTAP * 4));
                                }
                            };
#pragma unroll
                            for (int i = 0; i < kAhead && i < NTAP; ++i) fetch(i);
#pragma unroll
                            for (int i = 0; i < NTAP; ++i) {
                                if (i + kAhead < NTAP) fetch(i + kAhead);
                                asm volatile("" ::: "memory");
                                float f[4];
                                as4(b[i], f);
                                const float aN = a[i][0], aC = a[i][1], aP = a[i][2];
#pragma unroll
                                for (int v = 0; v < 4; ++v) {
                                    accN[v] = fmaf(aN, f[v], accN[v]);
                                    accC[v] = fmaf(aC, f[v], accC[v]);
                                    accP[v] = fmaf(aP, f[v], accP[v]);
                                }
                            }
                        };
                        bool face = false;
                        if constexpr (RAWR) {
                            int xsrc = xs - 1 + s;
                            xsrc = xsrc < 0 ? xsrc + P.nx : (xsrc >= P.nx ? xsrc - P.nx : xsrc);
                            face = xsrc == 0 || xsrc == P.nx - 1;
                            if (face) taps(std::true_type{}, xrank(xsrc, 1) * (NTAP * 4), xrank(xsrc, 0) * (NTAP * 4), xrank(xsrc, -1) * (NTAP * 4));
                        }
                        if (!face) taps(std::false_type{}, 0, 0, 0);
                    } else {
                        uint4 b[NTAP];
                        float a[NTAP][3];
#pragma unroll
                        for (int i = 0; i < NTAP; ++i) {
                            const int sN = 2 * NTAP + NTAP - 1 - i, sC = NTAP + NTAP - 1 - i, sP = NTAP - 1 - i;
                            const char* const vr = vb0 + tapv[i];
                            b[i] = make_uint4(0, 0, 0, 0);
                            a[i][0] = a[i][1] = a[i][2] = 0.f;
                            if (has(sN) || has(sC) || has(sP)) {
                                b[i] = *reinterpret_cast<const uint4*>(bb + tapb[i]);
                                if (has(sN)) a[i][0] = *reinterpret_cast<const float*>(vr + sN * 4);
                                if (has(sC)) a[i][1] = *reinterpret_cast<const float*>(vr + sC * 4);
                                if (has(sP)) a[i][2] = *reinterpret_cast<const float*>(vr + sP * 4);
                            }
                        }
#pragma unroll
                        for (int i = 0; i < NTAP; ++i) {
                            const int sN = 2 * NTAP + NTAP - 1 - i, sC = NTAP + NTAP - 1 - i, sP = NTAP - 1 - i;
                            float f[4];
                            as4(b[i], f);
                            if (has(sN)) {
#pragma unroll
                                for (int v = 0; v < 4; ++v) accN[v] = fmaf(a[i][0], f[v], accN[v]);
                            }
                            if (has(sC)) {
#pragma unroll
                                for (int v = 0; v < 4; ++v) accC[v] = fmaf(a[i][1], f[v], accC[v]);
                            }
                            if (has(sP)) {
#pragma unroll
                                for (int v = 0; v < 4; ++v) accP[v] = fmaf(a[i][2], f[v], accP[v]);
                            }
                        }
                    }
                }
            }
#pragma unroll
            for (int v = 0; v < 4; ++v) {
                done[v] = accP[v];
                accP[v] = accC[v];
                accC[v] = accN[v];
            }
            lat_step_sync();
        }
        flush();
    } else {
        constexpr bool XR = FULL && CL == 8 && NTAP == 9;
        auto slot_of = [&](int j) -> int { return XR ? (j < 3 ? 9 * j + c : (c < 3 ? 9 * c + 8 : NS)) : j * CL + c; };
        struct Own {
            uint4 row;
            int cls, start;
        };
        auto is_mid = [&](int x) -> bool { return x >= 1 && x <= P.nx - 2; };
        int kpk[(RJ + 3) / 4];
        int len_mid;
        {
            const int cm = crow >= 0 ? (int)P.rcls[row_of_x(1) + crow] : P.ident;
#pragma unroll
            for (int w = 0; w < (RJ + 3) / 4; ++w) kpk[w] = -1;
#pragma unroll
            for (int j = 0; j < RJ; ++j) {
                const int slot = slot_of(j);
                const int k = (slot < NS && has(slot)) ? (int)kidx_s[cm * 32 + slot] : 0xFF;
                kpk[j / 4] = (kpk[j / 4] & ~(0xFF << (8 * (j % 4)))) | (k << (8 * (j % 4)));
            }
            len_mid = kidx_s[cm * 32 + 31];
        }
        auto load_own = [&](int x, Own& o) {
            const int prow = row_of_x(x);
            o.cls = P.ident;
            o.start = 0;
            o.row = make_uint4(0, 0, 0, 0);
            if (crow >= 0) {
                if (!is_mid(x)) o.cls = P.rcls[prow + crow];
                if constexpr (PTR) o.start = P.rstart[prow + crow];
                o.row = *reinterpret_cast<const uint4*>(static_cast<const char*>(P.Own) + (int64_t)prow * P.ldown * 4 + cown);
            }
        };
        auto pin_own = [&](Own& o) {
            lat_pin(o.cls);
            if constexpr (PTR) lat_pin(o.start);
            lat_pin(o.row.x);
            lat_pin(o.row.y);
            lat_pin(o.row.z);
            lat_pin(o.row.w);
        };
        Own oP, oC, oN, old;
        oP.row = oC.row = make_uint4(0, 0, 0, 0);
        oP.cls = oC.cls = P.ident;
        oP.start = oC.start = 0;
        int x_own = xs;
        load_own(x_own, oN);
        pin_own(oN);
        x_own = wrap(x_own + 1, P.nx);
        old = oN;
        if (x_ok(0)) dma_ring(row_of_x(x_ring), 0);
        x_ring = wrap(x_ring + 1, P.nx);
        lat_step_sync();

        float rP[RJ], rC[RJ], rN[RJ];
#pragma unroll
        for (int j = 0; j < RJ; ++j) rP[j] = rC[j] = rN[j] = 0.f;
        constexpr bool PACKED = FULL && UNIF && (RPW * NS) % 4 == 0;
        constexpr int SP = PACKED ? NS * 4 : VP;
        const bool wave_packed = PACKED && P.tz % RPW == 0 && __all(crow >= 0);
        float* const st = reinterpret_cast<float*>(sm + P.o_vals + g * SP);
        const int own_const = PTR ? 0 : row_const(crow > 0 ? crow : 0);
        bool staged = false;
        int fl_start = 0, fl_len = 0;
        int x_out = xs;
        auto flush = [&]() {
            if constexpr (PACKED) {
                if (wave_packed) {
                    typedef float f4u __attribute__((ext_vector_type(4), aligned(4)));
                    const int first = __builtin_amdgcn_readfirstlane(fl_start);
                    if (lane < RPW * NS / 4) {
                        const float4 w4 = *reinterpret_cast<const float4*>(sm + P.o_vals + (wave * RPW) * SP + lane * 16);
                        f4u* const dst = reinterpret_cast<f4u*>(static_cast<float*>(P.gvals) + first) + lane;
                        f4u o = {w4.x, w4.y, w4.z, w4.w};
                        if (P.accumulate) {
                            const f4u prev = *dst;
                            o += prev;
                        }
                        __builtin_nontemporal_store(o, dst);
                    }
                    return;
                }
            }
            if (crow >= 0) {
                float* const go = static_cast<float*>(P.gvals) + fl_start;
                auto piece = [&](int k0) {
                    float4 w = *reinterpret_cast<const float4*>(st + k0);
                    if (k0 + 4 <= fl_len) {
                        typedef float f4u __attribute__((ext_vector_type(4), aligned(4)));
                        if (P.accumulate) {
                            const f4u prev = *reinterpret_cast<const f4u*>(go + k0);
                            w.x += prev.x, w.y += prev.y, w.z += prev.z, w.w += prev.w;
                        }
                        const f4u o = {w.x, w.y, w.z, w.w};
                        __builtin_nontemporal_store(o, reinterpret_cast<f4u*>(go + k0));
                    } else {
                        const float wv[4] = {w.x, w.y, w.z, w.w};
#pragma unroll
                        for (int j = 0; j < 4; ++j)
                            if (k0 + j < fl_len) go[k0 + j] = P.accumulate ? go[k0 + j] + wv[j] : wv[j];
                    }
                };
                if constexpr (UNIF) {
#pragma nounroll
                    for (int k0 = c * 4; k0 < fl_len; k0 += CL * 4) piece(k0);
                } else {
                    constexpr int kPieces = (SLOTS + CL * 4 - 1) / (CL * 4);
#pragma unroll
                    for (int it = 0; it < kPieces; ++it) {
                        const int k0 = c * 4 + it * CL * 4;
                        if (k0 < fl_len) piece(k0);
                    }
                }
            }
        };
        for (int s = 0; s <= L + 1; ++s) {
            if (s >= 1) {
                pin_own(old);
                oP = oC, oC = oN, oN = old;
            }
            if (staged) flush();
            staged = false;
            if (s + 1 <= L + 1 && x_ok(s + 1)) dma_ring(row_of_x(x_ring), (s + 1) & 1);
            x_ring = wrap(x_ring + 1, P.nx);
            if (s + 2 <= L) load_own(x_own, old);
            x_own = wrap(x_own + 1, P.nx);
            if (crow >= 0) {
              if (x_ok(s)) {
                const char* const bb = sm + (s & 1) * PB + cen;
                typedef float f2v __attribute__((ext_vector_type(2)));
                f2v nc[4];
                float op[4];
                {
                    float on[4], oc[4];
                    as4(oN.row, on);
                    as4(oC.row, oc);
                    as4(oP.row, op);
#pragma unroll
                    for (int v = 0; v < 4; ++v) nc[v] = f2v{on[v], oc[v]};
                }
                float pd[3][NTAP];
                if constexpr (FULL) {
                    uint4 b[NTAP];
                    constexpr int kAhead = 3;
                    auto tap_at = [&](int i) -> int { return XR && i < 8 ? tapx[i] : tapb[i]; };
#pragma unroll
                    for (int i = 0; i < kAhead && i < NTAP; ++i) b[i] = *reinterpret_cast<const uint4*>(bb + tap_at(i));
#pragma unroll
                    for (int i = 0; i < NTAP; ++i) {
                        if (i + kAhead < NTAP) b[i + kAhead] = *reinterpret_cast<const uint4*>(bb + tap_at(i + kAhead));
                        asm volatile("" ::: "memory");
                        float f[4];
                        as4(b[i], f);
                        const f2v f01 = {f[0], f[1]}, f23 = {f[2], f[3]};
                        f2v d2;
                        asm("v_pk_mul_f32 %0, %1, %2 op_sel_hi:[1,0]" : "=v"(d2) : "v"(nc[0]), "v"(f01));
                        asm("v_pk_fma_f32 %0, %1, %2, %0 op_sel:[0,1,0] op_sel_hi:[1,1,1]" : "+v"(d2) : "v"(nc[1]), "v"(f01));
                        asm("v_pk_fma_f32 %0, %1, %2, %0 op_sel_hi:[1,0,1]" : "+v"(d2) : "v"(nc[2]), "v"(f23));
                        asm("v_pk_fma_f32 %0, %1, %2, %0 op_sel:[0,1,0] op_sel_hi:[1,1,1]" : "+v"(d2) : "v"(nc[3]), "v"(f23));
                        float d;
                        asm("v_mul_f32 %0, %1, %2" : "=v"(d) : "v"(op[0]), "v"(f[0]));
#pragma unroll
                        for (int v = 1; v < 4; ++v) asm("v_fmac_f32 %0, %1, %2" : "+v"(d) : "v"(op[v]), "v"(f[v]));
                        pd[0][i] = d2.x, pd[1][i] = d2.y, pd[2][i] = d;
                    }
                } else {
                    uint4 b[NTAP];
#pragma unroll
                    for (int i = 0; i < NTAP; ++i) {
                        b[i] = make_uint4(0, 0, 0, 0);
                        if (has(i) || has(NTAP + i) || has(2 * NTAP + i)) {
                            b[i] = *reinterpret_cast<const uint4*>(bb + tapb[i]);
                        }
                    }
#pragma unroll
                    for (int i = 0; i < NTAP; ++i) {
                        float f[4];
                        as4(b[i], f);
                        pd[0][i] = pd[1][i] = pd[2][i] = 0.f;
                        if (has(i)) {
                            float d;
                            asm("v_mul_f32 %0, %1, %2" : "=v"(d) : "v"(nc[0].x), "v"(f[0]));
#pragma unroll
                            for (int v = 1; v < 4; ++v) asm("v_fmac_f32 %0, %1, %2" : "+v"(d) : "v"(nc[v].x), "v"(f[v]));
                            pd[0][i] = d;
                        }
                        if (has(NTAP + i)) {
                            float d;
                            asm("v_mul_f32 %0, %1, %2" : "=v"(d) : "v"(nc[0].y), "v"(f[0]));
#pragma unroll
                            for (int v = 1; v < 4; ++v) asm("v_fmac_f32 %0, %1, %2" : "+v"(d) : "v"(nc[v].y), "v"(f[v]));
                            pd[1][i] = d;
                        }
                        if (has(2 * NTAP + i)) {
                            float d;
                            asm("v_mul_f32 %0, %1, %2" : "=v"(d) : "v"(op[0]), "v"(f[0]));
#pragma unroll
                            for (int v = 1; v < 4; ++v) asm("v_fmac_f32 %0, %1, %2" : "+v"(d) : "v"(op[v]), "v"(f[v]));
                            pd[2][i] = d;
                        }
                    }
                }
                if constexpr (XR) {
                    auto halve8 = [&](const float (&R)[NTAP]) -> float {
                        const float u0 = R[0] + dpp_move<0xB1>(R[1]), u1 = R[2] + dpp_move<0xB1>(R[3]);
                        const float u2 = R[4] + dpp_move<0xB1>(R[5]), u3 = R[6] + dpp_move<0xB1>(R[7]);
                        const float v0 = u0 + dpp_move<0x4E>(u1), v1 = u2 + dpp_move<0x4E>(u3);
                        int y = __builtin_amdgcn_update_dpp(0, __float_as_int(v1), 0x104, 0xF, 0x5, false);
                        y = __builtin_amdgcn_update_dpp(y, __float_as_int(v1), 0x114, 0xF, 0xA, false);
                        return v0 + __int_as_float(y);
                    };
                    rN[0] = halve8(pd[0]);
                    rC[1] = halve8(pd[1]);
                    rP[2] = halve8(pd[2]);
                    const float t8 = group_sum_t8<3>(pd[0][8], pd[1][8], pd[2][8], 0.f, 0.f, 0.f, 0.f, 0.f, c);
                    rN[3] = c == 0 ? t8 : rN[3];
                    rC[3] = c == 1 ? t8 : rC[3];
                    rP[3] = c == 2 ? t8 : rP[3];
                } else if constexpr (CL == 8) {
                    lat_static_for<0, RJ>([&](auto J) {
                        constexpr int j = decltype(J)::value;
                        if (!FULL && ((mask >> (8 * j)) & 0xffu) == 0) return;
                        auto sl = [&](auto E) -> float {
                            constexpr int slot = 8 * j + decltype(E)::value;
                            if constexpr (slot < NS) return pd[slot / NTAP][slot % NTAP];
                            else return 0.f;
                        };
                        using std::integral_constant;
                        const float tot = group_sum_t8<(NS - 8 * j < 8 ? NS - 8 * j : 8)>(
                            sl(integral_constant<int, 0>{}), sl(integral_constant<int, 1>{}), sl(integral_constant<int, 2>{}), sl(integral_constant<int, 3>{}),
                            sl(integral_constant<int, 4>{}), sl(integral_constant<int, 5>{}), sl(integral_constant<int, 6>{}), sl(integral_constant<int, 7>{}), c);
#pragma unroll
                        for (int p = 0; p < 3; ++p) {
                            const int lo = (p * NTAP > 8 * j ? p * NTAP : 8 * j) - 8 * j, hi = ((p + 1) * NTAP < 8 * j + 8 ? (p + 1) * NTAP : 8 * j + 8) - 8 * j;
                            if (lo < hi) {
                                float& r = p == 0 ? rN[j] : (p == 1 ? rC[j] : rP[j]);
                                const bool whole = lo == 0 && (hi == 8 || 8 * j + hi == NS);
                                r = whole || (c >= lo && c < hi) ? tot : r;
                            }
                        }
                    });
                } else {
#pragma unroll
                    for (int p = 0; p < 3; ++p) {
#pragma unroll
                        for (int i = 0; i < NTAP; ++i) {
                            if (has(p * NTAP + i)) {
                                const float tot = group_sum<float, CL>(pd[p][i]);
                                const int slot = p * NTAP + i;
                                float& r = p == 0 ? rN[slot / CL] : (p == 1 ? rC[slot / CL] : rP[slot / CL]);
                                r = c == slot % CL ? tot : r;
                            }
                        }
                    }
                }
              }
                if (s >= 2) {
                    const bool mid = is_mid(x_out);
                    const bool plain = FULL && oP.cls == P.ident;
#pragma unroll
                    for (int j = 0; j < RJ; ++j) {
                        const int slot = slot_of(j);
                        if (slot < NS && has(slot)) {
                            int k;
                            if (mid) k = (kpk[j / 4] >> (8 * (j % 4))) & 0xFF;
                            else k = plain ? slot : (int)kidx_s[oP.cls * 32 + slot];
                            if (UNIF || k != 0xFF) st[k] = P.alpha * rP[j];
                        }
                    }
                    if constexpr (PTR) fl_start = oP.start;
                    else fl_start = plane_base(x_out) + plane_cx(x_out) * own_const;
                    fl_len = (FULL && UNIF) ? NS : (mid ? len_mid : (int)kidx_s[oP.cls * 32 + 31]);
                    staged = true;
                }
            }
            if (s >= 2) x_out = wrap(x_out + 1, P.nx);
#pragma unroll
            for (int j = 0; j < RJ; ++j) {
                rP[j] = rC[j];
                rC[j] = rN[j];
            }
            lat_step_sync();
        }
        if (staged) flush();
    }
}


inline int march_layout(MarchParams& P, int mode, int cl, int nt, int ntap) {
    if (P.ty <= 0 || P.tz <= 0 || P.ry < 0 || P.rz < 0 || P.ncls <= 0 || P.ncls > kMarchMaxCls || ntap != 9) return TSGU_ERR_BAD_ARG;
    const int HR = (P.ty + 2 * P.ry) * (P.tz + 2 * P.rz), NR = P.ty * P.tz, RB = cl * 16;
    const int VP = (3 * ntap + 3) / 4 * 4 * 4;
    const int NG = nt / cl;
    if ((int64_t)HR * cl > (int64_t)kMarchND * nt || NR > NG) return TSGU_ERR_TOO_LARGE;
    if (mode == kLatSpmmT && HR > 2 * NG) return TSGU_ERR_TOO_LARGE;
    int64_t o = 2 * (int64_t)HR * RB;
    P.o_vals = (int)o;
    if (mode == kLatSpmm) o += 4 * (int64_t)NR * VP;
    else if (mode == kLatSddmm) o += (int64_t)NR * VP;
    else o += 2 * (int64_t)HR * VP;
    P.o_tab = (int)o;
    o += P.ncls * 32;
    P.o_rows = (int)o;
    o += lat_round16((mode == kLatSpmmT ? HR : NR) * 4);
    if (o > kLatMaxLds) return TSGU_ERR_TOO_LARGE;
    P.lds_bytes = (int)o;
    return (int)o;
}

template <typename V, int CL, int MODE, int NT, uint32_t MASK, int ROWS>
int march_launch(const MarchParams& P, hipStream_t stream) {
    return launch_large_lds<march_kernel<V, CL, MODE, NT, 9, MASK, ROWS>>(current_device(), P.nblocks, NT, P.lds_bytes, kLatMaxLds, stream, P);
}

}
```

### torchsparsegradutils_amd/csrc/march_lower.hip

```cpp
#include "march_sets.h"

namespace tsgu {
int march_run_lower(int cl, const MarchParams& P, hipStream_t s) {
    switch (P.mask) {
        case kMarchLowerIncl: return march_subset_sddmm<kMarchLowerIncl>(cl, P, s);
        case kMarchLowerStrict: return march_subset_sddmm<kMarchLowerStrict>(cl, P, s);
        case kMarchLowerIncl & kMarchCross: return march_subset_sddmm<kMarchLowerIncl & kMarchCross>(cl, P, s);
        case kMarchLowerStrict & kMarchCross: return march_subset_sddmm<kMarchLowerStrict & kMarchCross>(cl, P, s);
    }
    return kMarchNotMine;
}
}
```

### torchsparsegradutils_amd/csrc/march_sets.h

```cpp
#pragma once

#include "march_impl.h"

namespace tsgu {

constexpr int kMarchNotMine = 1;
constexpr uint32_t kMarchCross = (1u << 4) | (1u << 10) | (1u << 12) | (1u << 13) | (1u << 14) | (1u << 16) | (1u << 22);
constexpr uint32_t kMarchLowerIncl = (1u << 14) - 1u, kMarchLowerStrict = (1u << 13) - 1u;
constexpr uint32_t kMarchUpperIncl = kBoxAll & ~kMarchLowerStrict, kMarchUpperStrict = kBoxAll & ~kMarchLowerIncl;

constexpr int kMarchSubsetThreads = 256;

int march_run_box(int mode, int cl, int threads, bool uni, const MarchParams& P, hipStream_t s);
int march_run_lower(int cl, const MarchParams& P, hipStream_t s);
int march_run_upper(int cl, const MarchParams& P, hipStream_t s);

constexpr bool march_is_triangular(uint32_t m) {
    return m == kMarchLowerIncl || m == kMarchLowerStrict || m == kMarchUpperIncl || m == kMarchUpperStrict ||
           m == (kMarchLowerIncl & kMarchCross) || m == (kMarchLowerStrict & kMarchCross) || m == (kMarchUpperIncl & kMarchCross) ||
           m == (kMarchUpperStrict & kMarchCross);
}
inline bool march_supported(int mode, uint32_t mask, bool uni, int threads) {
    if (mask == kBoxAll) return threads == 256 || threads == 512;
    return mode == kLatSddmm && !uni && threads == kMarchSubsetThreads && march_is_triangular(mask);
}

template <int MODE, int NT, uint32_t MASK, int ROWS>
int march_by_lanes(int cl, const MarchParams& P, hipStream_t s) {
    switch (cl) {
        case 4: return march_launch<float, 4, MODE, NT, MASK, ROWS>(P, s);
        case 8: return march_launch<float, 8, MODE, NT, MASK, ROWS>(P, s);
        case 16: return march_launch<float, 16, MODE, NT, MASK, ROWS>(P, s);
    }
    return TSGU_ERR_BAD_ARG;
}

constexpr int march_ragged_rows(uint32_t mask) { return mask == kBoxAll ? kRowsBox : kRowsPointer; }

template <uint32_t MASK>
int march_subset_sddmm(int cl, const MarchParams& P, hipStream_t s) {
    return march_by_lanes<kLatSddmm, kMarchSubsetThreads, MASK, kRowsPointer>(cl, P, s);
}

template <uint32_t MASK>
int march_both_sizes(int mode, int cl, int threads, bool uni, const MarchParams& P, hipStream_t s) {
#define TSGU_MARCH_CASE(M, T)                                                                   \
    if (mode == M && threads == T) {                                                            \
        if constexpr (MASK == kBoxAll && M != kLatSddmm) {                                      \
            if (uni && P.raw) return march_by_lanes<M, T, MASK, kRowsRaw>(cl, P, s);            \
        }                                                                                       \
        return uni ? march_by_lanes<M, T, MASK, kRowsUniform>(cl, P, s) : march_by_lanes<M, T, MASK, march_ragged_rows(MASK)>(cl, P, s); \
    }
    TSGU_MARCH_CASE(kLatSpmm, 256)
    TSGU_MARCH_CASE(kLatSpmm, 512)
    TSGU_MARCH_CASE(kLatSddmm, 256)
    TSGU_MARCH_CASE(kLatSddmm, 512)
    TSGU_MARCH_CASE(kLatSpmmT, 256)
    TSGU_MARCH_CASE(kLatSpmmT, 512)
#undef TSGU_MARCH_CASE
    return TSGU_ERR_BAD_ARG;
}

}
```

### torchsparsegradutils_amd/csrc/march_upper.hip

```cpp
#include "march_sets.h"

namespace tsgu {
int march_run_upper(int cl, const MarchParams& P, hipStream_t s) {
    switch (P.mask) {
        case kMarchUpperIncl: return march_subset_sddmm<kMarchUpperIncl>(cl, P, s);
        case kMarchUpperStrict: return march_subset_sddmm<kMarchUpperStrict>(cl, P, s);
        case kMarchUpperIncl & kMarchCross: return march_subset_sddmm<kMarchUpperIncl & kMarchCross>(cl, P, s);
        case kMarchUpperStrict & kMarchCross: return march_subset_sddmm<kMarchUpperStrict & kMarchCross>(cl, P, s);
    }
    return kMarchNotMine;
}
}
```

Measured before the change: 5574.

## Precompute plane-march block and halo index tables and hoist first ring DMA

Adds a per-config device table, built once on the host, that holds each workgroup's decoded tile, segment and item indices plus the y/z halo line indices and the packed tile coordinates. The march kernels get a TAB template variant that reads these instead of doing integer div/mod in the prologue. That variant also issues the first ring DMA earlier so it overlaps with row staging. The cost is extra template instantiations, a small plan-sized table, and scalar loads in place of arithmetic.

```diff
diff --git a/include/tsgu_hip.h b/include/tsgu_hip.h
--- a/include/tsgu_hip.h
+++ b/include/tsgu_hip.h
@@ -164,7 +164,11 @@
     const void* kidx;
     const void* rcls;
     const void* rstart;
+    const void* setup;
+    int64_t setup_bytes;
 } tsgu_march_plan;
+
+int64_t tsgu_march_setup_bytes(int64_t p, int nb, int ny, int nz, int ty, int tz, int nseg, int threads);
 
 int tsgu_march_supported(int mode, int mask, int uniform_len, int threads);
 int tsgu_march_lds_bytes(int mode, int vtype, int64_t p, int ty, int tz, int ry, int rz, int ncls, int threads);
diff --git a/torchsparsegradutils_amd/_backend.py b/torchsparsegradutils_amd/_backend.py
--- a/torchsparsegradutils_amd/_backend.py
+++ b/torchsparsegradutils_amd/_backend.py
@@ -110,6 +110,7 @@
     "tsgu_csr_sddmm_lattice": (_int, [_int, _ptr, _i64, _i64, _ptr, _i64, _ptr, _i64, _ptr, _dbl, _i64, _int, _ptr]),
     "tsgu_march_supported": (_int, [_int, _int, _int, _int]),
     "tsgu_march_lds_bytes": (_int, [_int, _int, _i64, _int, _int, _int, _int, _int, _int]),
+    "tsgu_march_setup_bytes": (_i64, [_i64, _int, _int, _int, _int, _int, _int, _int]),
     "tsgu_csr_spmm_march": (_int, [_int, _ptr, _int, _i64, _i64, _ptr, _ptr, _i64, _ptr, _i64, _i64, _int, _ptr]),
     "tsgu_csr_sddmm_march": (_int, [_int, _ptr, _i64, _i64, _ptr, _i64, _ptr, _i64, _ptr, _dbl, _int, _i64, _int, _ptr]),
     "tsgu_lattice_slots": (_int, []),
diff --git a/torchsparsegradutils_amd/_lattice.py b/torchsparsegradutils_amd/_lattice.py
--- a/torchsparsegradutils_amd/_lattice.py
+++ b/torchsparsegradutils_amd/_lattice.py
@@ -52,6 +52,11 @@
         for cfg in self._cfg.values():
             if cfg is not None:
                 total += cfg.rec.numel() * cfg.rec.element_size() + cfg.wlist.numel()
+        if self._march:
+            for cfg in self._march._cfg.values():
+                setup = getattr(cfg, "setup", None)
+                if setup is not None:
+                    total += setup.numel() * setup.element_size()
         return total
 
 
@@ -486,6 +491,14 @@
 _MARCH_WAVES_PER_CU = {0: 20, 1: 20, 2: 16}
 MARCH_SDDMM_SEGMENT_FACTOR = int(os.environ.get("TSGU_MARCH_SDDMM_SEGMENT_FACTOR", "1"))
 _MARCH_THREADS = {0: (256, 512), 1: (256, 512), 2: (512, 256), 3: (256,)}
+MARCH_SETUP = None
+
+
+def march_setup_mode() -> str:
+    mode = MARCH_SETUP or os.environ.get("TSGU_MARCH_SETUP", "table")
+    if mode not in ("table", "arith"):
+        raise ValueError(f"TSGU_MARCH_SETUP is 'table' or 'arith', not {mode!r}")
+    return mode
 _MARCH_HALO_COST = {0: 0.1, 1: 0.1, 2: 0.8, 3: 0.8}
 
 
@@ -496,7 +509,7 @@
 
 class MarchConfig:
 
-    __slots__ = ("mode", "ty", "tz", "nseg", "threads", "lds_bytes", "struct", "struct_addr", "ring", "cpl", "nloc", "tables", "col_tile")
+    __slots__ = ("mode", "ty", "tz", "nseg", "threads", "lds_bytes", "struct", "struct_addr", "ring", "cpl", "nloc", "tables", "col_tile", "setup")
     march = True
 
 
@@ -504,7 +517,8 @@
 
     _fields_ = ([(k, ctypes.c_int32) for k in ("nb", "nx", "ny", "nz", "ry", "rz", "ntap")] + [("tap_dy", ctypes.c_int32 * 9), ("tap_dz", ctypes.c_int32 * 9)]
                 + [(k, ctypes.c_int32) for k in ("ncls", "ident", "ty", "tz", "nseg", "threads")] + [("mask", ctypes.c_uint32)]
-                + [(k, ctypes.c_int32) for k in ("periodic", "uniform_len")] + [(k, ctypes.c_void_p) for k in ("kidx", "rcls", "rstart")])
+                + [(k, ctypes.c_int32) for k in ("periodic", "uniform_len")] + [(k, ctypes.c_void_p) for k in ("kidx", "rcls", "rstart", "setup")]
+                + [("setup_bytes", ctypes.c_int64)])
 
 
 MARCH_FULL = (1 << 27) - 1
@@ -543,6 +557,23 @@
     mt._cfg = {}
     plan._march = mt
     return mt
+
+
+def march_setup_tables(nb: int, ny: int, nz: int, ty: int, tz: int, nseg: int, threads: int, cl: int, periodic: int):
+    hy, hz = ty + 2, tz + 2
+    tiles_y, tiles_z = -(-ny // ty), -(-nz // tz)
+    w = torch.arange(nb * nseg * tiles_y * tiles_z, dtype=torch.int64)
+    block = torch.stack((w % tiles_z, w // tiles_z % tiles_y, w // (tiles_z * tiles_y) % nseg, w // (tiles_z * tiles_y * nseg)), 1)
+
+    def lines(tiles, t, n, per):
+        v = torch.arange(tiles, dtype=torch.int64)[:, None] * t - 1 + torch.arange(t + 2, dtype=torch.int64)[None, :]
+        inside = torch.ones_like(v, dtype=torch.bool) if per else (v >= 0) & (v < n)
+        return torch.where(inside, v % n, torch.full_like(v, -1))
+
+    r = torch.arange(hy * hz, dtype=torch.int64)
+    g = torch.arange(threads // cl, dtype=torch.int64)
+    parts = (block, lines(tiles_y, ty, ny, periodic >> 1 & 1), lines(tiles_z, tz, nz, periodic >> 2 & 1), r // hz | (r % hz) << 16, g // tz | (g % tz) << 16)
+    return tuple(t.to(torch.int32).contiguous() for t in parts)
 
 
 def march_config_for(plan: LatticePlan, mode: int, vtype: int, p: int, lds_bytes_fn, supported_fn=None) -> Optional[MarchConfig]:
@@ -614,9 +645,19 @@
         if (ENABLE_MARCH_RAW and plan.rcls.is_cuda and mt.full and mt.periodic == 7 and plan.uniform_len == 27
                 and (getattr(mt, "_line_ok", None) is not None or not torch.cuda.is_current_stream_capturing()) and linemarch_ok(plan, mt)):
             periodic |= 8
+        cfg.setup = None
+        if march_setup_mode() == "table" and plan.rcls.is_cuda:
+            host = torch.cat([t.reshape(-1) for t in march_setup_tables(plan.nb, plan.ny, plan.nz, ty, tz, nseg, threads, cl, mt.periodic)])
+            from . import _backend
+
+            want = int(_backend.load_library().tsgu_march_setup_bytes(pt, plan.nb, plan.ny, plan.nz, ty, tz, nseg, threads))
+            if want != host.numel() * 4:
+                raise RuntimeError(f"plane-march set-up table of {host.numel() * 4} bytes, the library expects {want}")
+            cfg.setup = host.to(plan.rcls.device)
         cfg.struct = _MarchPlanStruct(plan.nb, plan.nx, plan.ny, plan.nz, 1, 1, MARCH_TAPS, dy, dz, plan.ncls, mt.ident,
                                       ty, tz, nseg, threads, mt.mask, periodic, plan.uniform_len, mt.kidx.data_ptr(),
-                                      plan.rcls.data_ptr(), plan.rstart.data_ptr())
+                                      plan.rcls.data_ptr(), plan.rstart.data_ptr(),
+                                      cfg.setup.data_ptr() if cfg.setup is not None else None, cfg.setup.numel() * 4 if cfg.setup is not None else 0)
         cfg.struct_addr = ctypes.addressof(cfg.struct)
     mt._cfg[key] = cfg
     return cfg
diff --git a/torchsparsegradutils_amd/csrc/march.hip b/torchsparsegradutils_amd/csrc/march.hip
--- a/torchsparsegradutils_amd/csrc/march.hip
+++ b/torchsparsegradutils_amd/csrc/march.hip
@@ -55,7 +55,10 @@
     P.nnz = nnz;
     const int rc = march_layout(P, mode, cl, pl->threads, pl->ntap);
     if (rc < 0) return rc;
-    return set_workgroups(P, (int64_t)P.nb * P.nseg * P.tiles_y * P.tiles_z);
+    if (const int rw = set_workgroups(P, (int64_t)P.nb * P.nseg * P.tiles_y * P.tiles_z)) return rw;
+    const int64_t su_ints = march_setup_layout(P, cl, pl->threads);
+    P.setup = (pl->setup && pl->setup_bytes == su_ints * 4 && aligned16(pl->setup)) ? static_cast<const int*>(pl->setup) : nullptr;
+    return TSGU_OK;
 }
 
 template <int MODE>
@@ -63,8 +66,10 @@
     hipStream_t s = static_cast<hipStream_t>(stream);
     const bool uni = P.uniform > 0;
     if (!march_supported(MODE, P.mask, uni, threads)) return TSGU_ERR_BAD_ARG;
-    if (P.mask == kBoxAll) return march_run_box(MODE, cl, threads, uni, P, s);
-    const int rc = (P.mask & ~kMarchLowerIncl) == 0 ? march_run_lower(cl, P, s) : march_run_upper(cl, P, s);
+    const bool tab = P.setup != nullptr;
+    if (P.mask == kBoxAll) return tab ? march_run_box_tab(MODE, cl, threads, uni, P, s) : march_run_box(MODE, cl, threads, uni, P, s);
+    const int rc = (P.mask & ~kMarchLowerIncl) == 0 ? (tab ? march_run_lower_tab(cl, P, s) : march_run_lower(cl, P, s))
+                                                    : (tab ? march_run_upper_tab(cl, P, s) : march_run_upper(cl, P, s));
     return rc == kMarchNotMine ? TSGU_ERR_BAD_ARG : rc;
 }
 
@@ -75,6 +80,17 @@
 int tsgu_march_supported(int mode, int mask, int uniform_len, int threads) {
     if (mode < 0 || mode > kLatSpmmT || mask <= 0 || mask > (int)kBoxAll) return 0;
     return march_supported(mode, (uint32_t)mask, uniform_len > 0, threads) ? 1 : 0;
+}
+
+int64_t tsgu_march_setup_bytes(int64_t p, int nb, int ny, int nz, int ty, int tz, int nseg, int threads) {
+    const int cl = march_lanes(TSGU_F32, p);
+    if (cl == 0) return TSGU_ERR_BAD_DTYPE;
+    if (nb <= 0 || ny <= 0 || nz <= 0 || ty <= 0 || tz <= 0 || nseg <= 0 || (threads != 256 && threads != 512)) return TSGU_ERR_BAD_ARG;
+    MarchParams P{};
+    P.ty = ty, P.tz = tz, P.ry = 1, P.rz = 1;
+    P.tiles_y = (ny + ty - 1) / ty, P.tiles_z = (nz + tz - 1) / tz;
+    P.nblocks = (int64_t)nb * nseg * P.tiles_y * P.tiles_z;
+    return 4 * march_setup_layout(P, cl, threads);
 }
 
 int tsgu_march_lds_bytes(int mode, int vtype, int64_t p, int ty, int tz, int ry, int rz, int ncls, int threads) {
diff --git a/torchsparsegradutils_amd/csrc/march_box.hip b/torchsparsegradutils_amd/csrc/march_box.hip
--- a/torchsparsegradutils_amd/csrc/march_box.hip
+++ b/torchsparsegradutils_amd/csrc/march_box.hip
@@ -2,6 +2,6 @@
 
 namespace tsgu {
 int march_run_box(int mode, int cl, int threads, bool uni, const MarchParams& P, hipStream_t s) {
-    return march_both_sizes<kBoxAll>(mode, cl, threads, uni, P, s);
+    return march_both_sizes<kBoxAll, false>(mode, cl, threads, uni, P, s);
 }
 }
diff --git a/torchsparsegradutils_amd/csrc/march_box_tab.hip b/torchsparsegradutils_amd/csrc/march_box_tab.hip
--- /dev/null
+++ b/torchsparsegradutils_amd/csrc/march_box_tab.hip
@@ -0,0 +1,7 @@
+#include "march_sets.h"
+
+namespace tsgu {
+int march_run_box_tab(int mode, int cl, int threads, bool uni, const MarchParams& P, hipStream_t s) {
+    return march_both_sizes<kBoxAll, true>(mode, cl, threads, uni, P, s);
+}
+}
diff --git a/torchsparsegradutils_amd/csrc/march_impl.h b/torchsparsegradutils_amd/csrc/march_impl.h
--- a/torchsparsegradutils_amd/csrc/march_impl.h
+++ b/torchsparsegradutils_amd/csrc/march_impl.h
@@ -36,6 +36,8 @@
     float alpha;
     int64_t nblocks;
     int o_vals, o_stage, o_tab, o_rows, lds_bytes;
+    const int* setup;
+    int su_y, su_z, su_halo, su_tile;
 };
 
 template <bool NT_POLICY>
@@ -82,7 +84,7 @@
 
 enum MarchRows { kRowsPointer = 0, kRowsUniform = 1, kRowsBox = 2, kRowsRaw = 3 };
 
-template <typename V, int CL, int MODE, int NT, int NTAP, uint32_t MASK, int ROWS>
+template <typename V, int CL, int MODE, int NT, int NTAP, uint32_t MASK, int ROWS, bool TAB>
 __global__ __launch_bounds__(NT, 4) void march_kernel(const MarchParams P) {
     constexpr bool PTR = ROWS == kRowsPointer, RAWR = ROWS == kRowsRaw, UNIF = ROWS == kRowsUniform || RAWR, BOXA = ROWS == kRowsBox;
     static_assert(!RAWR || (MASK == kBoxAll && MODE != kLatSddmm), "raw value rows: SpMM / SpMMT of the whole box");
@@ -121,13 +123,20 @@
     constexpr uint32_t mask = MASK;
 
     const int64_t vblock = xcd_chunked_block(blockIdx.x, P.nblocks);
-    int64_t vb = vblock;
-    const int tzi = (int)(vb % P.tiles_z);
-    vb /= P.tiles_z;
-    const int tyi = (int)(vb % P.tiles_y);
-    vb /= P.tiles_y;
-    const int seg = (int)(vb % P.nseg);
-    const int item = (int)(vb / P.nseg);
+    int tzi, tyi, seg, item;
+    if constexpr (TAB) {
+        typedef int su_i4 __attribute__((ext_vector_type(4)));
+        const su_i4 bd = reinterpret_cast<const __attribute__((address_space(4))) su_i4*>((uintptr_t)P.setup)[vblock];
+        tzi = bd.x, tyi = bd.y, seg = bd.z, item = bd.w;
+    } else {
+        int64_t vb = vblock;
+        tzi = (int)(vb % P.tiles_z);
+        vb /= P.tiles_z;
+        tyi = (int)(vb % P.tiles_y);
+        vb /= P.tiles_y;
+        seg = (int)(vb % P.nseg);
+        item = (int)(vb / P.nseg);
+    }
     const int xs = seg * P.seg_len;
     const int L = P.seg_len < P.nx - xs ? P.seg_len : P.nx - xs;
     const int y0 = tyi * P.ty, z0 = tzi * P.tz;
@@ -139,6 +148,13 @@
         const bool in = (P.per_y || (unsigned)yy < (unsigned)P.ny) && (P.per_z || (unsigned)zz < (unsigned)P.nz);
         return in ? lat_mod(yy, P.ny) * P.nz + lat_mod(zz, P.nz) : -1;
     };
+    const int* const su_yrow = P.setup + P.su_y + tyi * HY;
+    const int* const su_zrow = P.setup + P.su_z + tzi * HZ;
+    auto halo_row_tab = [&](int hr) -> int {
+        const int pk = P.setup[P.su_halo + hr];
+        const int yy = su_yrow[pk & 0xffff], zz = su_zrow[pk >> 16];
+        return (yy | zz) >= 0 ? yy * P.nz + zz : -1;
+    };
 
     auto cnt1 = [](int t, int n, int per) -> int { return per ? 3 : 3 - (t == 0) - (t == n - 1); };
     auto pre1 = [](int t, int per) -> int { return per ? 3 * t : 3 * t - (t > 0); };
@@ -161,6 +177,31 @@
         else return row_of_x(x) * (FULL ? NS : P.uniform);
     };
 
+    const uint32_t ldsb = (uint32_t)P.lds_ * 4u;
+    uint32_t roff[kMarchND];
+    const int ring_pieces = HR * CL;
+    const char* const Sb = static_cast<const char*>(P.S);
+    auto dma_ring = [&](int prow, int slot) {
+        const char* const pbase = Sb + (int64_t)__builtin_amdgcn_readfirstlane(prow) * ldsb;
+        const unsigned base = sbase + (unsigned)(slot * PB) + (unsigned)(wave * kWave * 16);
+#pragma unroll
+        for (int d = 0; d < kMarchND; ++d) {
+            if (d * NT < ring_pieces) {
+                if (roff[d] != kLatNone) lat_dma16<false>(pbase, roff[d], base + (unsigned)(d * NT * 16));
+            }
+        }
+    };
+    int x_ring = xs == 0 ? P.nx - 1 : xs - 1;
+    if constexpr (TAB) {
+#pragma unroll
+        for (int d = 0; d < kMarchND; ++d) {
+            const int e = d * NT + tid;
+            const int hrow_in_plane = e < ring_pieces ? halo_row_tab(e / CL) : -1;
+            roff[d] = hrow_in_plane >= 0 ? (uint32_t)hrow_in_plane * ldsb + (uint32_t)c * 16u : kLatNone;
+        }
+        if (x_ok(0)) dma_ring(row_of_x(x_ring), 0);
+    }
+
     const int staged_rows = MODE == kLatSpmmT ? HR : NR;
     {
         const int* src = reinterpret_cast<const int*>(P.kidx);
@@ -170,10 +211,20 @@
         for (int r = tid; r < staged_rows; r += NT) {
             int v;
             if constexpr (MODE == kLatSpmmT) {
-                const int hy = r / HZ, hz = r - hy * HZ;
-                v = halo_row(hy, hz);
+                if constexpr (TAB) {
+                    v = halo_row_tab(r);
+                } else {
+                    const int hy = r / HZ, hz = r - hy * HZ;
+                    v = halo_row(hy, hz);
+                }
             } else {
-                const int ly = r / P.tz, lz = r - ly * P.tz;
+                int ly, lz;
+                if constexpr (TAB) {
+                    const int pk = P.setup[P.su_tile + r];
+                    ly = pk & 0xffff, lz = pk >> 16;
+                } else {
+                    ly = r / P.tz, lz = r - ly * P.tz;
+                }
                 v = (y0 + ly < P.ny && z0 + lz < P.nz) ? (y0 + ly) * P.nz + z0 + lz : -1;
             }
             rows[r] = v;
@@ -185,16 +236,15 @@
     constexpr bool rawv = RAWR;
     auto xrank = [&](int x, int d) -> int { return x == 0 ? (d < 0 ? 2 : d) : (x == P.nx - 1 ? (d > 0 ? 0 : d + 2) : d + 1); };
 
-    const uint32_t ldsb = (uint32_t)P.lds_ * 4u;
-    uint32_t roff[kMarchND];
-    const int ring_pieces = HR * CL;
-#pragma unroll
-    for (int d = 0; d < kMarchND; ++d) {
-        const int e = d * NT + tid;
-        const int hr = e / CL;
-        const int hy = hr / HZ, hz = hr - hy * HZ;
-        const int hrow_in_plane = e < ring_pieces ? halo_row(hy, hz) : -1;
-        roff[d] = hrow_in_plane >= 0 ? (uint32_t)hrow_in_plane * ldsb + (uint32_t)c * 16u : kLatNone;
+    if constexpr (!TAB) {
+#pragma unroll
+        for (int d = 0; d < kMarchND; ++d) {
+            const int e = d * NT + tid;
+            const int hr = e / CL;
+            const int hy = hr / HZ, hz = hr - hy * HZ;
+            const int hrow_in_plane = e < ring_pieces ? halo_row(hy, hz) : -1;
+            roff[d] = hrow_in_plane >= 0 ? (uint32_t)hrow_in_plane * ldsb + (uint32_t)c * 16u : kLatNone;
+        }
     }
     if (!(P.per_y && P.per_z)) {
 #pragma unroll
@@ -216,7 +266,13 @@
         if constexpr (MODE == kLatSpmm) {
             for (int e = tid; e < NR * SLOTS; e += NT) {
                 const int r = e / SLOTS, slot = e - r * SLOTS;
-                const int ry_ = r / P.tz, rz_ = r - ry_ * P.tz;
+                int ry_, rz_;
+                if constexpr (TAB) {
+                    const int pk = P.setup[P.su_tile + r];
+                    ry_ = pk & 0xffff, rz_ = pk >> 16;
+                } else {
+                    ry_ = r / P.tz, rz_ = r - ry_ * P.tz;
+                }
                 const int yy = y0 + ry_ + (slot / 3) % 3 - 1, zz = z0 + rz_ + slot % 3 - 1;
                 const bool beyond = (!P.per_y && (unsigned)yy >= (unsigned)P.ny) || (!P.per_z && (unsigned)zz >= (unsigned)P.nz);
                 if (slot < NS && beyond) {
@@ -226,7 +282,13 @@
             }
         }
     }
-    const int ly = g / P.tz, lz = g - ly * P.tz;
+    int ly, lz;
+    if constexpr (TAB) {
+        const int pk = P.setup[P.su_tile + g];
+        ly = pk & 0xffff, lz = pk >> 16;
+    } else {
+        ly = g / P.tz, lz = g - ly * P.tz;
+    }
     const bool ok = g < NR && y0 + ly < P.ny && z0 + lz < P.nz;
     const int crow = ok ? (y0 + ly) * P.nz + z0 + lz : -1;
     const int hrow = (ly + P.ry) * HZ + lz + P.rz;
@@ -292,20 +354,9 @@
         }
     }
 
-    const char* const Sb = static_cast<const char*>(P.S);
     const char* const valb = static_cast<const char*>(P.val);
     const uint32_t val_bytes = (uint32_t)(P.nnz * 4);
 
-    auto dma_ring = [&](int prow, int slot) {
-        const char* const pbase = Sb + (int64_t)prow * ldsb;
-        const unsigned base = sbase + (unsigned)(slot * PB) + (unsigned)(wave * kWave * 16);
-#pragma unroll
-        for (int d = 0; d < kMarchND; ++d) {
-            if (d * NT < ring_pieces) {
-                if (roff[d] != kLatNone) lat_dma16<false>(pbase, roff[d], base + (unsigned)(d * NT * 16));
-            }
-        }
-    };
     auto stage_vals = [&](int pbase, int pcx, bool mid, int xv, unsigned region, const int (&cls)[NPASS], const int (&stt)[NPASS]) {
         if constexpr (MODE != kLatSddmm) {
 #pragma unroll
@@ -436,8 +487,6 @@
         f[0] = __uint_as_float(raw.x), f[1] = __uint_as_float(raw.y), f[2] = __uint_as_float(raw.z), f[3] = __uint_as_float(raw.w);
     };
 
-    int x_ring = lat_mod(xs - 1, P.nx);
-
     if constexpr (MODE == kLatSpmm || MODE == kLatSpmmT) {
         constexpr int VB = MODE == kLatSpmm ? 4 : 2;
         const int vbuf = (MODE == kLatSpmm ? NR : HR) * VP;
@@ -462,7 +511,9 @@
             load_cls(row_of_x(x_val), cls, stt);
             pin_cls(cls, stt);
         }
-        if (x_ok(0)) dma_ring(row_of_x(x_ring), 0);
+        if constexpr (!TAB) {
+            if (x_ok(0)) dma_ring(row_of_x(x_ring), 0);
+        }
         if (x_ok(first_val)) stage_vals(vbase, vcx, is_mid(x_val), x_val, (unsigned)(P.o_vals + (MODE == kLatSpmm ? 1 : 0) * vbuf), cls, stt);
         x_ring = wrap(x_ring + 1, P.nx);
         next_val_plane();
@@ -706,7 +757,9 @@
         pin_own(oN);
         x_own = wrap(x_own + 1, P.nx);
         old = oN;
-        if (x_ok(0)) dma_ring(row_of_x(x_ring), 0);
+        if constexpr (!TAB) {
+            if (x_ok(0)) dma_ring(row_of_x(x_ring), 0);
+        }
         x_ring = wrap(x_ring + 1, P.nx);
         lat_step_sync();
 
@@ -965,9 +1018,23 @@
     return (int)o;
 }
 
-template <typename V, int CL, int MODE, int NT, uint32_t MASK, int ROWS>
+inline int64_t march_setup_layout(MarchParams& P, int cl, int nt) {
+    const int HY = P.ty + 2 * P.ry, HZ = P.tz + 2 * P.rz;
+    int64_t o = 4 * P.nblocks;
+    P.su_y = (int)o;
+    o += (int64_t)P.tiles_y * HY;
+    P.su_z = (int)o;
+    o += (int64_t)P.tiles_z * HZ;
+    P.su_halo = (int)o;
+    o += (int64_t)HY * HZ;
+    P.su_tile = (int)o;
+    o += nt / cl;
+    return o;
+}
+
+template <typename V, int CL, int MODE, int NT, uint32_t MASK, int ROWS, bool TAB>
 int march_launch(const MarchParams& P, hipStream_t stream) {
-    return launch_large_lds<march_kernel<V, CL, MODE, NT, 9, MASK, ROWS>>(current_device(), P.nblocks, NT, P.lds_bytes, kLatMaxLds, stream, P);
+    return launch_large_lds<march_kernel<V, CL, MODE, NT, 9, MASK, ROWS, TAB>>(current_device(), P.nblocks, NT, P.lds_bytes, kLatMaxLds, stream, P);
 }
 
 }
diff --git a/torchsparsegradutils_amd/csrc/march_lower.hip b/torchsparsegradutils_amd/csrc/march_lower.hip
--- a/torchsparsegradutils_amd/csrc/march_lower.hip
+++ b/torchsparsegradutils_amd/csrc/march_lower.hip
@@ -3,10 +3,10 @@
 namespace tsgu {
 int march_run_lower(int cl, const MarchParams& P, hipStream_t s) {
     switch (P.mask) {
-        case kMarchLowerIncl: return march_subset_sddmm<kMarchLowerIncl>(cl, P, s);
-        case kMarchLowerStrict: return march_subset_sddmm<kMarchLowerStrict>(cl, P, s);
-        case kMarchLowerIncl & kMarchCross: return march_subset_sddmm<kMarchLowerIncl & kMarchCross>(cl, P, s);
-        case kMarchLowerStrict & kMarchCross: return march_subset_sddmm<kMarchLowerStrict & kMarchCross>(cl, P, s);
+        case kMarchLowerIncl: return march_subset_sddmm<kMarchLowerIncl, false>(cl, P, s);
+        case kMarchLowerStrict: return march_subset_sddmm<kMarchLowerStrict, false>(cl, P, s);
+        case kMarchLowerIncl & kMarchCross: return march_subset_sddmm<kMarchLowerIncl & kMarchCross, false>(cl, P, s);
+        case kMarchLowerStrict & kMarchCross: return march_subset_sddmm<kMarchLowerStrict & kMarchCross, false>(cl, P, s);
     }
     return kMarchNotMine;
 }
diff --git a/torchsparsegradutils_amd/csrc/march_lower_tab.hip b/torchsparsegradutils_amd/csrc/march_lower_tab.hip
--- /dev/null
+++ b/torchsparsegradutils_amd/csrc/march_lower_tab.hip
@@ -0,0 +1,13 @@
+#include "march_sets.h"
+
+namespace tsgu {
+int march_run_lower_tab(int cl, const MarchParams& P, hipStream_t s) {
+    switch (P.mask) {
+        case kMarchLowerIncl: return march_subset_sddmm<kMarchLowerIncl, true>(cl, P, s);
+        case kMarchLowerStrict: return march_subset_sddmm<kMarchLowerStrict, true>(cl, P, s);
+        case kMarchLowerIncl & kMarchCross: return march_subset_sddmm<kMarchLowerIncl & kMarchCross, true>(cl, P, s);
+        case kMarchLowerStrict & kMarchCross: return march_subset_sddmm<kMarchLowerStrict & kMarchCross, true>(cl, P, s);
+    }
+    return kMarchNotMine;
+}
+}
diff --git a/torchsparsegradutils_amd/csrc/march_sets.h b/torchsparsegradutils_amd/csrc/march_sets.h
--- a/torchsparsegradutils_amd/csrc/march_sets.h
+++ b/torchsparsegradutils_amd/csrc/march_sets.h
@@ -14,6 +14,9 @@
 int march_run_box(int mode, int cl, int threads, bool uni, const MarchParams& P, hipStream_t s);
 int march_run_lower(int cl, const MarchParams& P, hipStream_t s);
 int march_run_upper(int cl, const MarchParams& P, hipStream_t s);
+int march_run_box_tab(int mode, int cl, int threads, bool uni, const MarchParams& P, hipStream_t s);
+int march_run_lower_tab(int cl, const MarchParams& P, hipStream_t s);
+int march_run_upper_tab(int cl, const MarchParams& P, hipStream_t s);
 
 constexpr bool march_is_triangular(uint32_t m) {
     return m == kMarchLowerIncl || m == kMarchLowerStrict || m == kMarchUpperIncl || m == kMarchUpperStrict ||
@@ -25,31 +28,31 @@
     return mode == kLatSddmm && !uni && threads == kMarchSubsetThreads && march_is_triangular(mask);
 }
 
-template <int MODE, int NT, uint32_t MASK, int ROWS>
+template <int MODE, int NT, uint32_t MASK, int ROWS, bool TAB>
 int march_by_lanes(int cl, const MarchParams& P, hipStream_t s) {
     switch (cl) {
-        case 4: return march_launch<float, 4, MODE, NT, MASK, ROWS>(P, s);
-        case 8: return march_launch<float, 8, MODE, NT, MASK, ROWS>(P, s);
-        case 16: return march_launch<float, 16, MODE, NT, MASK, ROWS>(P, s);
+        case 4: return march_launch<float, 4, MODE, NT, MASK, ROWS, TAB>(P, s);
+        case 8: return march_launch<float, 8, MODE, NT, MASK, ROWS, TAB>(P, s);
+        case 16: return march_launch<float, 16, MODE, NT, MASK, ROWS, TAB>(P, s);
     }
     return TSGU_ERR_BAD_ARG;
 }
 
 constexpr int march_ragged_rows(uint32_t mask) { return mask == kBoxAll ? kRowsBox : kRowsPointer; }
 
-template <uint32_t MASK>
+template <uint32_t MASK, bool TAB>
 int march_subset_sddmm(int cl, const MarchParams& P, hipStream_t s) {
-    return march_by_lanes<kLatSddmm, kMarchSubsetThreads, MASK, kRowsPointer>(cl, P, s);
+    return march_by_lanes<kLatSddmm, kMarchSubsetThreads, MASK, kRowsPointer, TAB>(cl, P, s);
 }
 
-template <uint32_t MASK>
+template <uint32_t MASK, bool TAB>
 int march_both_sizes(int mode, int cl, int threads, bool uni, const MarchParams& P, hipStream_t s) {
 #define TSGU_MARCH_CASE(M, T)                                                                   \
     if (mode == M && threads == T) {                                                            \
         if constexpr (MASK == kBoxAll && M != kLatSddmm) {                                      \
-            if (uni && P.raw) return march_by_lanes<M, T, MASK, kRowsRaw>(cl, P, s);            \
+            if (uni && P.raw) return march_by_lanes<M, T, MASK, kRowsRaw, TAB>(cl, P, s);            \
         }                                                                                       \
-        return uni ? march_by_lanes<M, T, MASK, kRowsUniform>(cl, P, s) : march_by_lanes<M, T, MASK, march_ragged_rows(MASK)>(cl, P, s); \
+        return uni ? march_by_lanes<M, T, MASK, kRowsUniform, TAB>(cl, P, s) : march_by_lanes<M, T, MASK, march_ragged_rows(MASK), TAB>(cl, P, s); \
     }
     TSGU_MARCH_CASE(kLatSpmm, 256)
     TSGU_MARCH_CASE(kLatSpmm, 512)
diff --git a/torchsparsegradutils_amd/csrc/march_upper.hip b/torchsparsegradutils_amd/csrc/march_upper.hip
--- a/torchsparsegradutils_amd/csrc/march_upper.hip
+++ b/torchsparsegradutils_amd/csrc/march_upper.hip
@@ -3,10 +3,10 @@
 namespace tsgu {
 int march_run_upper(int cl, const MarchParams& P, hipStream_t s) {
     switch (P.mask) {
-        case kMarchUpperIncl: return march_subset_sddmm<kMarchUpperIncl>(cl, P, s);
-        case kMarchUpperStrict: return march_subset_sddmm<kMarchUpperStrict>(cl, P, s);
-        case kMarchUpperIncl & kMarchCross: return march_subset_sddmm<kMarchUpperIncl & kMarchCross>(cl, P, s);
-        case kMarchUpperStrict & kMarchCross: return march_subset_sddmm<kMarchUpperStrict & kMarchCross>(cl, P, s);
+        case kMarchUpperIncl: return march_subset_sddmm<kMarchUpperIncl, false>(cl, P, s);
+        case kMarchUpperStrict: return march_subset_sddmm<kMarchUpperStrict, false>(cl, P, s);
+        case kMarchUpperIncl & kMarchCross: return march_subset_sddmm<kMarchUpperIncl & kMarchCross, false>(cl, P, s);
+        case kMarchUpperStrict & kMarchCross: return march_subset_sddmm<kMarchUpperStrict & kMarchCross, false>(cl, P, s);
     }
     return kMarchNotMine;
 }
diff --git a/torchsparsegradutils_amd/csrc/march_upper_tab.hip b/torchsparsegradutils_amd/csrc/march_upper_tab.hip
--- /dev/null
+++ b/torchsparsegradutils_amd/csrc/march_upper_tab.hip
@@ -0,0 +1,13 @@
+#include "march_sets.h"
+
+namespace tsgu {
+int march_run_upper_tab(int cl, const MarchParams& P, hipStream_t s) {
+    switch (P.mask) {
+        case kMarchUpperIncl: return march_subset_sddmm<kMarchUpperIncl, true>(cl, P, s);
+        case kMarchUpperStrict: return march_subset_sddmm<kMarchUpperStrict, true>(cl, P, s);
+        case kMarchUpperIncl & kMarchCross: return march_subset_sddmm<kMarchUpperIncl & kMarchCross, true>(cl, P, s);
+        case kMarchUpperStrict & kMarchCross: return march_subset_sddmm<kMarchUpperStrict & kMarchCross, true>(cl, P, s);
+    }
+    return kMarchNotMine;
+}
+}
```

After: 5539. Within noise of the previous version (-0.6%).
